# Joao-M-Silva/padel_analytics

Hardware: AMD Instinct MI355X
Metric: frames/sec (all trackers) on 1280x720 (higher is better)
Workload: dtype f32-equivalent (h2: fp16 pairs h + m/2048, 2 or 3 f16 MFMA products per multiply, fp32 accumulate)

## Files before the change

padel_analytics_amd/csrc/conv_1x1_h2s.hip:

```cpp
#include "h2_common.h"

namespace padel {

namespace {

__device__ __forceinline__ unsigned hs_off(int p, int q) { return (unsigned)(p * 64 + ((q ^ (((p >> 2) & 1) << 1)) << 4)); }

typedef int hs_i32x4 __attribute__((ext_vector_type(4)));

}

#ifndef PADEL_HS_AWIN
#define PADEL_HS_AWIN D
#endif
template <int WC, int PROBE = 0, int D = 2, int WR = 2>
__global__ void __launch_bounds__(64 * WR * WC, 2) conv_h2s_kernel(const ConvArgs a) {
    constexpr int MF = 4, NF = 3, NSET = D + 1;
    constexpr int kSPlaneB = 64 * WR * 64;
    constexpr int kSStageB = 2 * kSPlaneB;
    constexpr int kSStages = WC == 2 ? 5 : 9;
    constexpr int kSAhead = kSStages - 1;
    constexpr int NA = 8 / (2 * WC) * 2;
    static_assert(WR == 2 || WC == 4, "64-pixel tiles: one span per wave");
    __shared__ __attribute__((aligned(16))) float lds[(kSStages * kSStageB) / 4];
    char* const ldsb = reinterpret_cast<char*>(lds);
    const int tid = threadIdx.x;
    const int lane = tid & 63;
    const int wave = __builtin_amdgcn_readfirstlane(tid >> 6);
    const int wr = WR == 2 ? (wave & 1) : 0, wc = WR == 2 ? (wave >> 1) : wave;
    const int lr = lane & 15, lq = lane >> 4;

    const int nmt = a.n_mtiles, nnt = a.n_ntiles;
    const int bid = blockIdx.x;
    const int q8 = nmt >> 3, r8 = nmt & 7, xcd = bid & 7, idx = bid >> 3;
    const int mloc = idx / nnt, nt = idx - mloc * nnt;
    if (mloc >= q8 + (xcd < r8 ? 1 : 0)) return;
    const int mt = (xcd < r8 ? xcd * (q8 + 1) : r8 * (q8 + 1) + (xcd - r8) * q8) + mloc;
    const int m0 = mt * (64 * WR);
    const int f0 = nt * WC * NF;
    const int nch = a.cin >> 5;

    const long long pix_b = (long long)a.in_cs * 4;
    const char* const in0 = reinterpret_cast<const char*>(a.in + a.in_choff) + (long long)m0 * pix_b;
    i32x4 rsrcA = make_rsrc3(in0);
    {
        const long long left = ((long long)a.M - m0) * pix_b;
        rsrcA[2] = (int)(left > 0x7FFFFFFFll ? 0x7FFFFFFFll : left);
    }
    const int p_q = (lane & 3) ^ (((lane >> 4) & 1) << 1);
    const unsigned p_piece = (unsigned)((p_q >> 1) * 64 + (p_q & 1) * 16);
    unsigned voA[2];
#pragma unroll
    for (int k = 0; k < 2; ++k) voA[k] = (unsigned)(((wave + 4 * k) * 16 + (lane >> 2)) * (unsigned)pix_b) + p_piece;
    unsigned voL[2];
#pragma unroll
    for (int k = 0; k < 2; ++k) voL[k] = (unsigned)((wave * 16 + 8 * k + (lane >> 3)) * (unsigned)pix_b) + (unsigned)(lane & 7) * 16u;
    hs_i32x4 sink[2] = {};
    unsigned voQ[2];
#pragma unroll
    for (int k = 0; k < 2; ++k) voQ[k] = (unsigned)(wave * 2048 + k * 1024 + lane * 16);
    const unsigned lp0 = __builtin_amdgcn_readfirstlane((unsigned)(uintptr_t)lds);
    const unsigned lpw = __builtin_amdgcn_readfirstlane(lp0 + (unsigned)wave * 1024u);
#define PADEL_HS_REQA(SB_, K_)                                                                                    \
    if constexpr (PROBE != 3) {                                                                                   \
        const unsigned so_ = (unsigned)(K_) * 128u;                                                               \
        const unsigned lb_ = lpw + (unsigned)(SB_);                                                               \
        i32x4 rs_ = rsrcA;                                                                                        \
        if ((int)(K_) >= nch) rs_[2] = 0;                                                                         \
        if constexpr (PROBE == 4) { dma3<0>(voL[0], rs_, so_, lb_); dma3<kSPlaneB>(voL[1], rs_, so_, lb_); }      \
        else if constexpr (PROBE == 6) {                                                                          \
            asm volatile("buffer_load_dwordx4 %0, %1, %2, %3 offen" : "=v"(sink[0]) : "v"(voA[0]), "s"(rs_), "s"(so_) : "memory"); \
            asm volatile("buffer_load_dwordx4 %0, %1, %2, %3 offen" : "=v"(sink[1]) : "v"(voA[0]), "s"(rs_), "s"(so_ + 32u) : "memory"); \
        }                                                                                                         \
        else if constexpr (PROBE == 5) { dma3<0>(voQ[0], rs_, so_ * 128u, lb_); dma3<kSPlaneB>(voQ[1], rs_, so_ * 128u, lb_); } \
        else {                                                                                                    \
        dma3<0>(voA[0], rs_, so_, lb_); if constexpr (WC == 2) dma3<4096>(voA[1], rs_, so_, lb_);                 \
        dma3<kSPlaneB>(voA[0], rs_, so_ + 32u, lb_); if constexpr (WC == 2) dma3<kSPlaneB + 4096>(voA[1], rs_, so_ + 32u, lb_); \
        }                                                                                                         \
    }

    const unsigned fragb = (unsigned)nch * 2048u;
    const unsigned voffW = (unsigned)lane * 16u;
    i32x4 rsrcW[NF];
#pragma unroll
    for (int j = 0; j < NF; ++j) {
        const int frag = min(f0 + NF * wc + j, a.n16 - 1);
        rsrcW[j] = make_rsrc3(reinterpret_cast<const char*>(a.wr) + (long long)frag * fragb);
    }
    hs_i32x4 w[NSET][NF];
#define PADEL_HS_LOADW(SET_, K_)                                                                                  \
    if constexpr (PROBE != 2 && PROBE < 4 || PROBE == 7) {                                                        \
        const unsigned so_ = (unsigned)(K_) * 2048u;                                                              \
        if (PROBE == 7 && wr == 1) rsrcW[0][2] = rsrcW[1][2] = rsrcW[2][2] = 0;      \
        _Pragma("unroll") for (int j = 0; j < NF; ++j)                                                            \
            asm volatile("buffer_load_dwordx4 %0, %1, %2, %3 offen" : "=v"(w[SET_][j]) : "v"(voffW), "s"(rsrcW[j]), "s"(so_) : "memory"); \
    }
#define PADEL_HS_WAITW(SET_, N_)                                                                                  \
    asm volatile("s_waitcnt vmcnt(%3)" : "+v"(w[SET_][0]), "+v"(w[SET_][1]), "+v"(w[SET_][2]) : "n"(PROBE == 2 || (PROBE >= 4 && PROBE != 7) ? ((N_) == 0 ? 0 : (PADEL_HS_AWIN) * NA) : PROBE == 3 ? (N_) * NF / (NF + NA) : (N_)) : "memory")

    const unsigned abase = hs_off(64 * wr + lr, lq);
    f32x4 acc[MF][NF], part[MF][NF], cross[MF][NF];
#pragma unroll
    for (int f = 0; f < MF; ++f)
#pragma unroll
        for (int j = 0; j < NF; ++j) { acc[f][j] = (f32x4){0.f, 0.f, 0.f, 0.f}; part[f][j] = acc[f][j]; cross[f][j] = acc[f][j]; }
    h16x8 ah[MF], am[MF];
#define PADEL_HS_MFMA(F_, SET_)                                                                                   \
    do {                                                                                                          \
        _Pragma("unroll") for (int j = 0; j < NF; ++j)                                                            \
            cross[F_][j] = __builtin_amdgcn_mfma_f32_16x16x32_f16(__builtin_bit_cast(h16x8, w[SET_][j]), am[F_], cross[F_][j], 0, 0, 0); \
        _Pragma("unroll") for (int j = 0; j < NF; ++j)                                                            \
            part[F_][j] = __builtin_amdgcn_mfma_f32_16x16x32_f16(__builtin_bit_cast(h16x8, w[SET_][j]), ah[F_], part[F_][j], 0, 0, 0); \
        __builtin_amdgcn_sched_barrier(0);                                                                        \
    } while (0)
#define PADEL_HS_STEP(K_, SET_)                                                                                   \
    do {                                                                                                          \
        PADEL_HS_LOADW(((SET_) + D) % NSET, (K_) + D);                                                            \
        PADEL_HS_WAITW(SET_, D * (NF + NA));                                                                      \
        __builtin_amdgcn_s_barrier();              \
        asm volatile("" ::: "memory");                                                                            \
        PADEL_HS_REQA(s_wr, (K_) + kSAhead);                                                                      \
        __builtin_amdgcn_sched_barrier(0);                                                                        \
        if constexpr (PROBE == 0) {                                                                               \
            const char* p_ = ldsb + abase + s_rd;                                                                 \
            _Pragma("unroll") for (int f = 0; f < MF; ++f) {                                                      \
                ah[f] = *reinterpret_cast<const h16x8*>(p_ + f * 1024);                                           \
                am[f] = *reinterpret_cast<const h16x8*>(p_ + f * 1024 + kSPlaneB);                                \
            }                                                                                                     \
        }                                                                                                         \
        __builtin_amdgcn_sched_barrier(0);                                                                        \
        if constexpr (PROBE == 0) { PADEL_HS_MFMA(0, SET_); PADEL_HS_MFMA(1, SET_); PADEL_HS_MFMA(2, SET_); PADEL_HS_MFMA(3, SET_); } \
        if (++kblk == 9) {                         \
            kblk = 0;                                                                                             \
            _Pragma("unroll") for (int f = 0; f < MF; ++f)                                                        \
                _Pragma("unroll") for (int j = 0; j < NF; ++j) { acc[f][j] += part[f][j]; part[f][j] = (f32x4){0.f, 0.f, 0.f, 0.f}; } \
        }                                                                                                         \
        s_wr = s_rd;                                                                                              \
        s_rd = s_rd + (unsigned)kSStageB == (unsigned)(kSStages * kSStageB) ? 0u : s_rd + (unsigned)kSStageB;     \
    } while (0)

    int kblk = 0;
    unsigned s_rd = 0, s_wr = (unsigned)((kSStages - 1) * kSStageB);
    static_assert(kSAhead >= D, "the ring is at least as deep as the weight look-ahead");
#pragma unroll
    for (int k = 0; k < kSAhead - D; ++k) PADEL_HS_REQA(k * kSStageB, k);
#pragma unroll
    for (int i = 0; i < D; ++i) {
        PADEL_HS_LOADW(i, i);
        PADEL_HS_REQA((kSAhead - D + i) * kSStageB, kSAhead - D + i);
    }
#pragma unroll 1
    for (int k = 0; k < nch; k += NSET) {
        PADEL_HS_STEP(k, 0);
#pragma unroll
        for (int i = 1; i < NSET; ++i)
            if (k + i < nch) PADEL_HS_STEP(k + i, i);
    }
    if (kblk != 0) {
#pragma unroll
        for (int f = 0; f < MF; ++f)
#pragma unroll
            for (int j = 0; j < NF; ++j) acc[f][j] += part[f][j];
    }
#pragma unroll
    for (int i = 0; i < NSET; ++i) PADEL_HS_WAITW(i, 0);
    if constexpr (PROBE == 6) asm volatile("" :: "v"(sink[0]), "v"(sink[1]));
#undef PADEL_HS_STEP
#undef PADEL_HS_MFMA
#undef PADEL_HS_WAITW
#undef PADEL_HS_LOADW
#undef PADEL_HS_REQA

    int mpix[MF];
#pragma unroll
    for (int f = 0; f < MF; ++f) {
        const int m = m0 + 64 * wr + 16 * f + lr;
        mpix[f] = m < a.M ? m : -1;
    }
    const int fw = f0 + NF * wc;
    const bool fast = m0 + 64 * WR <= a.M && (fw + NF) * 16 <= a.cout && (((a.out_choff | a.out_cs) & 3) == 0) &&
                      (!a.res || (((a.res_choff | a.res_cs) & 3) == 0));
    if (fw < a.n16) h2_epilogue<MF, NF>(a, acc, cross, mpix, fw, lq, fast);
}

template <int PROBE = 0, int WR = 2>
__global__ void __launch_bounds__(256 * WR, 2) conv_h2s3_kernel(const ConvArgs a) {
    constexpr int MF = 4, NF = 3, WC = 4;
    constexpr int kSPlaneB = 64 * WR * 64, kSStageB = 2 * kSPlaneB;
    constexpr int kSStages = 9, kSAhead = 8, NA = 2;
    __shared__ __attribute__((aligned(16))) float lds[(kSStages * kSStageB) / 4];
    char* const ldsb = reinterpret_cast<char*>(lds);
    const int tid = threadIdx.x;
    const int lane = tid & 63;
    const int wave = __builtin_amdgcn_readfirstlane(tid >> 6);
    const int wr = WR == 2 ? (wave & 1) : 0, wc = WR == 2 ? (wave >> 1) : wave;
    const int lr = lane & 15, lq = lane >> 4;

    const int nmt = a.n_mtiles, nnt = a.n_ntiles;
    const int bid = blockIdx.x;
    const int q8 = nmt >> 3, r8 = nmt & 7, xcd = bid & 7, idx = bid >> 3;
    const int mloc = idx / nnt, nt = idx - mloc * nnt;
    if (mloc >= q8 + (xcd < r8 ? 1 : 0)) return;
    const int mt = (xcd < r8 ? xcd * (q8 + 1) : r8 * (q8 + 1) + (xcd - r8) * q8) + mloc;
    const int m0 = mt * (64 * WR);
    const int f0 = nt * WC * NF;
    const int nch = a.cin >> 5;
    const int HoWo = a.Ho * a.Wo;

    const long long pix_b = (long long)a.in_cs * 4;
    long long lin0;
    {
        const int n = fastdiv3(m0, a.howo_magic, a.howo_shift);
        const int rem = m0 - n * HoWo;
        const int oy = fastdiv3(rem, a.wo_magic, a.wo_shift), ox = rem - oy * a.Wo;
        lin0 = ((long long)n * a.H + (2 * oy - 1)) * a.W + (2 * ox - 1);
    }
    const i32x4 rsrcA = make_rsrc3(reinterpret_cast<const char*>(a.in + a.in_choff) + lin0 * pix_b);
    const int p_q = (lane & 3) ^ (((lane >> 4) & 1) << 1);
    const unsigned p_piece = (unsigned)((p_q >> 1) * 64 + (p_q & 1) * 16);
    unsigned voA, vbits = 0;
    {
        const int m = m0 + wave * 16 + (lane >> 2);
        const bool mv = m < a.M;
        const int mc = mv ? m : m0;
        const int n = fastdiv3(mc, a.howo_magic, a.howo_shift);
        const int rem = mc - n * HoWo;
        const int oy = fastdiv3(rem, a.wo_magic, a.wo_shift), ox = rem - oy * a.Wo;
        const int iy0 = 2 * oy - 1, ix0 = 2 * ox - 1;
        const long long lin = ((long long)n * a.H + iy0) * a.W + ix0;
        voA = (unsigned)((lin - lin0) * pix_b) + p_piece;
        if (mv) {
#pragma unroll
            for (int k = 0; k < 3; ++k) {
                vbits |= ((unsigned)(iy0 + k) < (unsigned)a.H ? 1u : 0u) << k;
                vbits |= ((unsigned)(ix0 + k) < (unsigned)a.W ? 8u : 0u) << k;
            }
        }
    }
    const unsigned rowb = (unsigned)a.W * (unsigned)pix_b;
    const unsigned lp0 = __builtin_amdgcn_readfirstlane((unsigned)(uintptr_t)lds);
    const unsigned lpw = __builtin_amdgcn_readfirstlane(lp0 + (unsigned)wave * 1024u);
#define PADEL_HS3_REQA(SB_, CH_, TAP_)                                                                            \
    do {                                                                                                          \
        constexpr int ky_ = (TAP_) % 3, kx_ = (TAP_) / 3;                                                         \
        constexpr unsigned need_ = (1u << ky_) | (8u << kx_);                                                     \
        const unsigned so_ = (unsigned)(CH_) * 128u + (unsigned)ky_ * rowb + (unsigned)kx_ * (unsigned)pix_b;     \
        const unsigned lb_ = lpw + (unsigned)(SB_);                                                               \
        i32x4 rs_ = rsrcA;                                                                                        \
        if ((int)(CH_) >= nch) rs_[2] = 0;                                                                        \
        const unsigned vo_ = (vbits & need_) == need_ ? voA : kOOR3;                                              \
        dma3<0>(vo_, rs_, so_, lb_); dma3<kSPlaneB>(vo_, rs_, so_ + 32u, lb_);                                    \
    } while (0)

    const unsigned fragb = (unsigned)(nch * 9) * 2048u;
    const unsigned voffW = (unsigned)lane * 16u;
    i32x4 rsrcW[NF];
#pragma unroll
    for (int j = 0; j < NF; ++j) {
        const int frag = min(f0 + NF * wc + j, a.n16 - 1);
        rsrcW[j] = make_rsrc3(reinterpret_cast<const char*>(a.wr) + (long long)frag * fragb);
    }
    hs_i32x4 w[3][NF];
    unsigned s_kw = 0;
#define PADEL_HS3_LOADW(SET_, TT_)                                                                                \
    do {                                                                                                          \
        const unsigned so_ = s_kw + (unsigned)((TT_) * 2048);                                                     \
        _Pragma("unroll") for (int j = 0; j < NF; ++j)                                                            \
            asm volatile("buffer_load_dwordx4 %0, %1, %2, %3 offen" : "=v"(w[SET_][j]) : "v"(voffW), "s"(rsrcW[j]), "s"(so_) : "memory"); \
    } while (0)
#define PADEL_HS3_WAITW(SET_, N_)                                                                                 \
    asm volatile("s_waitcnt vmcnt(%3)" : "+v"(w[SET_][0]), "+v"(w[SET_][1]), "+v"(w[SET_][2]) : "n"(N_) : "memory")

    const unsigned abase = hs_off(64 * wr + lr, lq);
    f32x4 acc[MF][NF], part[MF][NF], cross[MF][NF];
#pragma unroll
    for (int f = 0; f < MF; ++f)
#pragma unroll
        for (int j = 0; j < NF; ++j) { acc[f][j] = (f32x4){0.f, 0.f, 0.f, 0.f}; part[f][j] = acc[f][j]; cross[f][j] = acc[f][j]; }
    h16x8 ah[MF], am[MF];
#define PADEL_HS3_MFMA(F_, SET_)                                                                                  \
    do {                                                                                                          \
        _Pragma("unroll") for (int j = 0; j < NF; ++j)                                                            \
            cross[F_][j] = __builtin_amdgcn_mfma_f32_16x16x32_f16(__builtin_bit_cast(h16x8, w[SET_][j]), am[F_], cross[F_][j], 0, 0, 0); \
        _Pragma("unroll") for (int j = 0; j < NF; ++j)                                                            \
            part[F_][j] = __builtin_amdgcn_mfma_f32_16x16x32_f16(__builtin_bit_cast(h16x8, w[SET_][j]), ah[F_], part[F_][j], 0, 0, 0); \
        __builtin_amdgcn_sched_barrier(0);                                                                        \
    } while (0)
#define PADEL_HS3_STEP(T_)                                                                                        \
    do {                                                                                                          \
        PADEL_HS3_LOADW(((T_) + 2) % 3, (T_) + 2);                                                                \
        PADEL_HS3_WAITW((T_) % 3, 2 * NF + 2 * NA);                                                               \
        __builtin_amdgcn_s_barrier();                                                                             \
        asm volatile("" ::: "memory");                                                                            \
        PADEL_HS3_REQA(s_wr, c + ((T_) >= 1 ? 1 : 0), ((T_) + 8) % 9);                                            \
        __builtin_amdgcn_sched_barrier(0);                                                                        \
        if constexpr (PROBE == 0) {                                                                               \
            const char* p_ = ldsb + abase + s_rd;                                                                 \
            _Pragma("unroll") for (int f = 0; f < MF; ++f) {                                                      \
                ah[f] = *reinterpret_cast<const h16x8*>(p_ + f * 1024);                                           \
                am[f] = *reinterpret_cast<const h16x8*>(p_ + f * 1024 + kSPlaneB);                                \
            }                                                                                                     \
        }                                                                                                         \
        __builtin_amdgcn_sched_barrier(0);                                                                        \
        if constexpr (PROBE == 0) { PADEL_HS3_MFMA(0, (T_) % 3); PADEL_HS3_MFMA(1, (T_) % 3); PADEL_HS3_MFMA(2, (T_) % 3); PADEL_HS3_MFMA(3, (T_) % 3); } \
        s_wr = s_rd;                                                                                              \
        s_rd = s_rd + (unsigned)kSStageB == (unsigned)(kSStages * kSStageB) ? 0u : s_rd + (unsigned)kSStageB;     \
    } while (0)

    unsigned s_rd = 0, s_wr = (unsigned)((kSStages - 1) * kSStageB);
    PADEL_HS3_REQA(0 * kSStageB, 0, 0); PADEL_HS3_REQA(1 * kSStageB, 0, 1);
    PADEL_HS3_REQA(4 * kSStageB, 0, 4); PADEL_HS3_REQA(5 * kSStageB, 0, 5); PADEL_HS3_REQA(6 * kSStageB, 0, 6); PADEL_HS3_REQA(7 * kSStageB, 0, 7);
    PADEL_HS3_LOADW(0, 0);
    PADEL_HS3_REQA(2 * kSStageB, 0, 2);
    PADEL_HS3_LOADW(1, 1);
    PADEL_HS3_REQA(3 * kSStageB, 0, 3);
#pragma unroll 1
    for (int c = 0; c < nch; ++c) {
        PADEL_HS3_STEP(0); PADEL_HS3_STEP(1); PADEL_HS3_STEP(2); PADEL_HS3_STEP(3); PADEL_HS3_STEP(4);
        PADEL_HS3_STEP(5); PADEL_HS3_STEP(6); PADEL_HS3_STEP(7); PADEL_HS3_STEP(8);
#pragma unroll
        for (int f = 0; f < MF; ++f)
#pragma unroll
            for (int j = 0; j < NF; ++j) { acc[f][j] += part[f][j]; part[f][j] = (f32x4){0.f, 0.f, 0.f, 0.f}; }
        s_kw += 9u * 2048u;
    }
    PADEL_HS3_WAITW(0, 0); PADEL_HS3_WAITW(1, 0); PADEL_HS3_WAITW(2, 0);
#undef PADEL_HS3_STEP
#undef PADEL_HS3_MFMA
#undef PADEL_HS3_WAITW
#undef PADEL_HS3_LOADW
#undef PADEL_HS3_REQA

    int mpix[MF];
#pragma unroll
    for (int f = 0; f < MF; ++f) {
        const int m = m0 + 64 * wr + 16 * f + lr;
        mpix[f] = m < a.M ? m : -1;
    }
    const int fw = f0 + NF * wc;
    const bool fast = m0 + 64 * WR <= a.M && (fw + NF) * 16 <= a.cout && (((a.out_choff | a.out_cs) & 3) == 0) &&
                      (!a.res || (((a.res_choff | a.res_cs) & 3) == 0));
    if (fw < a.n16) h2_epilogue<MF, NF>(a, acc, cross, mpix, fw, lq, fast);
}

bool conv_h2s3_supported(const ConvArgs& a) {
    return a.w_single && a.wr && a.ksize == 3 && a.stride == 2 && (a.cin & 31) == 0 && a.cin >= 32 && a.w != nullptr && !a.in2 &&
           a.Ho <= (a.H + 1) / 2 && a.Wo <= (a.W + 1) / 2 && (long long)4 * a.W * a.in_cs * 4 < 0x3FFFFFFFll;
}

hipError_t launch_conv_h2s3(const ConvArgs& a_in, hipStream_t s, bool m64) {
    if (!conv_h2s3_supported(a_in)) return hipErrorNotSupported;
    ConvArgs a = a_in;
    a.n_mtiles = m64 ? (a.M + 63) / 64 : (a.M + 127) / 128;
    a.n_ntiles = (a.n16 + 11) / 12;
    dim3 grid(8u * (unsigned)((a.n_mtiles + 7) / 8) * (unsigned)a.n_ntiles, 1, 1);
    if (m64) {
        if (a.tune & 64) hipLaunchKernelGGL((conv_h2s3_kernel<1, 1>), grid, dim3(256), 0, s, a);
        else hipLaunchKernelGGL((conv_h2s3_kernel<0, 1>), grid, dim3(256), 0, s, a);
        return hipGetLastError();
    }
    if (a.tune & 64) hipLaunchKernelGGL((conv_h2s3_kernel<1>), grid, dim3(512), 0, s, a);
    else hipLaunchKernelGGL((conv_h2s3_kernel<0>), grid, dim3(512), 0, s, a);
    return hipGetLastError();
}

bool conv_h2s_supported(const ConvArgs& a) {
    return a.w_single && a.wr && a.ksize == 1 && a.stride == 1 && (a.cin & 31) == 0 && a.cin >= 64 && a.Ho == a.H && a.Wo == a.W && a.w != nullptr &&
           !a.in2 && (long long)128 * a.in_cs * 4 < 0x7FFFFFFFll;
}

hipError_t launch_conv_h2s(const ConvArgs& a_in, bool nf12, hipStream_t s, bool m64) {
    if (!conv_h2s_supported(a_in)) return hipErrorNotSupported;
    ConvArgs a = a_in;
    if (nf12 && m64) {
        a.n_mtiles = (a.M + 63) / 64;
        a.n_ntiles = (a.n16 + 11) / 12;
        dim3 grid(8u * (unsigned)((a.n_mtiles + 7) / 8) * (unsigned)a.n_ntiles, 1, 1);
        if (a.tune & 64) hipLaunchKernelGGL((conv_h2s_kernel<4, 1, 2, 1>), grid, dim3(256), 0, s, a);
        else hipLaunchKernelGGL((conv_h2s_kernel<4, 0, 2, 1>), grid, dim3(256), 0, s, a);
        return hipGetLastError();
    }
    a.n_mtiles = (a.M + 127) / 128;
    const bool wide = nf12;
    a.n_ntiles = wide ? (a.n16 + 11) / 12 : (a.n16 + 5) / 6;
    dim3 grid(8u * (unsigned)((a.n_mtiles + 7) / 8) * (unsigned)a.n_ntiles, 1, 1);
    if (wide) {
        static bool attr = false;
        if (!attr) {
            (void)hipFuncSetAttribute(reinterpret_cast<const void*>(conv_h2s_kernel<4, 0>), hipFuncAttributeMaxDynamicSharedMemorySize, 0);
            attr = true;
        }
        if ((a.tune & 64) && (a.tune & 4096)) hipLaunchKernelGGL((conv_h2s_kernel<4, 7>), grid, dim3(512), 0, s, a);
        else if ((a.tune & 64) && (a.tune & 2048)) hipLaunchKernelGGL((conv_h2s_kernel<4, 6>), grid, dim3(512), 0, s, a);
        else if ((a.tune & 64) && (a.tune & 1024)) hipLaunchKernelGGL((conv_h2s_kernel<4, 5>), grid, dim3(512), 0, s, a);
        else if ((a.tune & 64) && (a.tune & 256) && (a.tune & 512)) hipLaunchKernelGGL((conv_h2s_kernel<4, 4>), grid, dim3(512), 0, s, a);
        else if ((a.tune & 64) && (a.tune & 256)) hipLaunchKernelGGL((conv_h2s_kernel<4, 2>), grid, dim3(512), 0, s, a);
        else if ((a.tune & 64) && (a.tune & 512)) hipLaunchKernelGGL((conv_h2s_kernel<4, 3>), grid, dim3(512), 0, s, a);
        else if (a.tune & 64) hipLaunchKernelGGL((conv_h2s_kernel<4, 1>), grid, dim3(512), 0, s, a);
        else if (a.tune & 8) hipLaunchKernelGGL((conv_h2s_kernel<4, 0, 4>), grid, dim3(512), 0, s, a);
        else hipLaunchKernelGGL((conv_h2s_kernel<4, 0, 2>), grid, dim3(512), 0, s, a);
    } else if (a.tune & 64) hipLaunchKernelGGL((conv_h2s_kernel<2, 1>), grid, dim3(256), 0, s, a);
    else if (a.tune & 8) hipLaunchKernelGGL((conv_h2s_kernel<2, 0, 3>), grid, dim3(256), 0, s, a);
    else hipLaunchKernelGGL((conv_h2s_kernel<2, 0, 2>), grid, dim3(256), 0, s, a);
    return hipGetLastError();
}

}
```

padel_analytics_amd/csrc/conv_patch_h2v.hip:

```cpp
#include "h2_common.h"

namespace padel {

namespace {

constexpr int kVPW = 18, kVNPix = 18 * 18;
constexpr int kVSpans = (kVNPix + 15) / 16;
constexpr int kVPlaneB = kVSpans * 1024;
constexpr int kVTSpans = (kVNPix + 31) / 32;
constexpr int kVTPlaneB = kVTSpans * 1024;

__device__ __forceinline__ unsigned hv_tail_off(int p, int s) { return (unsigned)(p * 32 + ((s ^ ((p >> 3) & 1)) << 4)); }

typedef int hv_i32x4 __attribute__((ext_vector_type(4)));

}

template <int NF, bool CHUNK, bool TAIL, bool WS>
__global__ void __launch_bounds__(256, 2) conv_h2v_kernel(const ConvArgs a) {
    static_assert(CHUNK || TAIL, "cin = 32 CHUNK + 16 TAIL");
    static_assert(WS || NF <= 2, "three products: 2 fragments per wave (6 register sets of 4 VGPRs per step)");
    constexpr int MF = 4;
    constexpr int PATCH_B = (CHUNK ? 2 * kVPlaneB : 0);
    constexpr int TPATCH_B = (TAIL ? 2 * kVTPlaneB : 0);
    constexpr int NSTEPS = (CHUNK ? 9 : 0) + (TAIL ? 5 : 0);
    constexpr int NPL = WS ? 1 : 2;
    constexpr int NW = NF * NPL;
    __shared__ __attribute__((aligned(16))) float lds[(PATCH_B + TPATCH_B) / 4];
    char* const ldsb = reinterpret_cast<char*>(lds);
    const int tid = threadIdx.x;
    const int lane = tid & 63;
    const int wave = __builtin_amdgcn_readfirstlane(tid >> 6);
    const int lr = lane & 15, lq = lane >> 4;

    const int nmt = a.n_mtiles, nnt = a.n_ntiles;
    const int bid = blockIdx.x;
    const int q8 = nmt >> 3, r8 = nmt & 7, xcd = bid & 7, idx = bid >> 3;
    const int mloc = idx / nnt, nt = idx - mloc * nnt;
    if (mloc >= q8 + (xcd < r8 ? 1 : 0)) return;
    const int mt = (xcd < r8 ? xcd * (q8 + 1) : r8 * (q8 + 1) + (xcd - r8) * q8) + mloc;
    const int txN = (a.Wo + 15) >> 4, tyN = (a.Ho + 15) >> 4;
    const int tpi = tyN * txN;
    const int n = mt / tpi, rt = mt - n * tpi;
    const int ty = rt / txN, tx = rt - ty * txN;
    const int y0 = ty * 16, x0 = tx * 16;
    const int f0 = nt * NF;

    const float* const in0 = a.in + (((long long)n * a.H + (y0 - 1)) * a.W + (x0 - 1)) * a.in_cs + a.in_choff;
    const i32x4 rsrcP = make_rsrc3(in0);
    const unsigned lp0 = __builtin_amdgcn_readfirstlane((unsigned)(uintptr_t)lds);

    if constexpr (CHUNK) {
        const int p_lane = lane >> 2;
        const int p_q = (lane & 3) ^ (((lane >> 4) & 1) << 1);
        const unsigned p_piece = (unsigned)((p_q >> 1) * 64 + (p_q & 1) * 16);
#define PADEL_HV_PSPAN(S_)                                                                                        \
        if (((S_) & 3) == wave) {                                                                                 \
            const int pp_ = (S_) * 16 + p_lane;                                                                   \
            const int py_ = pp_ / kVPW, px_ = pp_ - py_ * kVPW;                                                   \
            const bool ok_ = pp_ < kVNPix && (unsigned)(y0 - 1 + py_) < (unsigned)a.H && (unsigned)(x0 - 1 + px_) < (unsigned)a.W; \
            const unsigned vo_ = ok_ ? (unsigned)((py_ * a.W + px_) * a.in_cs * 4) + p_piece : kOOR3;             \
            dma3<(S_) * 1024>(vo_, rsrcP, 0u, lp0);                                                               \
            dma3<kVPlaneB + (S_) * 1024>(vo_, rsrcP, 32u, lp0);                                                   \
        }
        PADEL_HV_PSPAN(0) PADEL_HV_PSPAN(1) PADEL_HV_PSPAN(2) PADEL_HV_PSPAN(3) PADEL_HV_PSPAN(4) PADEL_HV_PSPAN(5) PADEL_HV_PSPAN(6)
        PADEL_HV_PSPAN(7) PADEL_HV_PSPAN(8) PADEL_HV_PSPAN(9) PADEL_HV_PSPAN(10) PADEL_HV_PSPAN(11) PADEL_HV_PSPAN(12) PADEL_HV_PSPAN(13)
        PADEL_HV_PSPAN(14) PADEL_HV_PSPAN(15) PADEL_HV_PSPAN(16) PADEL_HV_PSPAN(17) PADEL_HV_PSPAN(18) PADEL_HV_PSPAN(19) PADEL_HV_PSPAN(20)
#undef PADEL_HV_PSPAN
    }
    if constexpr (TAIL) {
        const int t_lane = lane >> 1;
        const unsigned t_piece = (unsigned)(((lane & 1) ^ ((lane >> 4) & 1)) * 16);
        const unsigned t_so = CHUNK ? 128u : 0u;
#define PADEL_HV_TSPAN(S_)                                                                                        \
        if (((S_) & 3) == ((wave + 1) & 3)) {                                                                     \
            const int pp_ = (S_) * 32 + t_lane;                                                                   \
            const int py_ = pp_ / kVPW, px_ = pp_ - py_ * kVPW;                                                   \
            const bool ok_ = pp_ < kVNPix && (unsigned)(y0 - 1 + py_) < (unsigned)a.H && (unsigned)(x0 - 1 + px_) < (unsigned)a.W; \
            const unsigned vo_ = ok_ ? (unsigned)((py_ * a.W + px_) * a.in_cs * 4) + t_piece : kOOR3;             \
            dma3<PATCH_B + (S_) * 1024>(vo_, rsrcP, t_so, lp0);                                                   \
            dma3<PATCH_B + kVTPlaneB + (S_) * 1024>(vo_, rsrcP, t_so + 32u, lp0);                                 \
        }
        PADEL_HV_TSPAN(0) PADEL_HV_TSPAN(1) PADEL_HV_TSPAN(2) PADEL_HV_TSPAN(3) PADEL_HV_TSPAN(4) PADEL_HV_TSPAN(5)
        PADEL_HV_TSPAN(6) PADEL_HV_TSPAN(7) PADEL_HV_TSPAN(8) PADEL_HV_TSPAN(9) PADEL_HV_TSPAN(10)
#undef PADEL_HV_TSPAN
    }

    constexpr unsigned fragb = (unsigned)NSTEPS * 2048u;
    const unsigned voffW = (unsigned)lane * 16u;
    i32x4 rsrcW[NF];
#pragma unroll
    for (int j = 0; j < NF; ++j) {
        const int frag = min(f0 + j, a.n16 - 1);
        rsrcW[j] = make_rsrc3(reinterpret_cast<const char*>(a.wr) + (long long)frag * fragb);
    }
    hv_i32x4 w[3][NF], wm[3][WS ? 1 : NF];
#define PADEL_HV_LOADW(ST_)                                                                                       \
    do {                                                                                                          \
        const unsigned so_ = (unsigned)((ST_) * 2048);                                                            \
        _Pragma("unroll") for (int j = 0; j < NF; ++j) {                                                          \
            asm volatile("buffer_load_dwordx4 %0, %1, %2, %3 offen"                                               \
                         : "=v"(w[(ST_) % 3][j]) : "v"(voffW), "s"(rsrcW[j]), "s"(so_) : "memory");               \
            if constexpr (!WS)                                                                                    \
                asm volatile("buffer_load_dwordx4 %0, %1, %2, %3 offen offset:1024"                               \
                             : "=v"(wm[(ST_) % 3][j]) : "v"(voffW), "s"(rsrcW[j]), "s"(so_) : "memory");          \
        }                                                                                                         \
    } while (0)
#define PADEL_HV_WAITW(ST_, N_)                                                                                   \
    do {                                                                                                          \
        if constexpr (NF == 3)                                                                                    \
            asm volatile("s_waitcnt vmcnt(%3)" : "+v"(w[(ST_) % 3][0]), "+v"(w[(ST_) % 3][1]), "+v"(w[(ST_) % 3][2]) : "n"(N_) : "memory"); \
        else if constexpr (NF == 2 && WS)                                                                         \
            asm volatile("s_waitcnt vmcnt(%2)" : "+v"(w[(ST_) % 3][0]), "+v"(w[(ST_) % 3][1]) : "n"(N_) : "memory"); \
        else if constexpr (NF == 2)                                                                               \
            asm volatile("s_waitcnt vmcnt(%4)" : "+v"(w[(ST_) % 3][0]), "+v"(w[(ST_) % 3][1]), "+v"(wm[(ST_) % 3][0]), "+v"(wm[(ST_) % 3][WS ? 0 : NF - 1]) \
                         : "n"(N_) : "memory");                                                                   \
        else if constexpr (WS)                                                                                    \
            asm volatile("s_waitcnt vmcnt(%1)" : "+v"(w[(ST_) % 3][0]) : "n"(N_) : "memory");                     \
        else                                                                                                      \
            asm volatile("s_waitcnt vmcnt(%2)" : "+v"(w[(ST_) % 3][0]), "+v"(wm[(ST_) % 3][0]) : "n"(N_) : "memory"); \
    } while (0)

    unsigned rbase[8];
    if constexpr (CHUNK) {
#pragma unroll
        for (int r = 0; r < 8; ++r) {
            const int p0 = 4 * wave * kVPW + lr;
            rbase[r] = (unsigned)(p0 * 64 + ((lq ^ ((((p0 + r) >> 2) & 1) << 1)) << 4));
        }
    }
    const int rd_pix = 4 * wave * kVPW + lr;

    f32x4 acc[MF][NF], part[MF][NF], cross[MF][NF];
#pragma unroll
    for (int f = 0; f < MF; ++f)
#pragma unroll
        for (int j = 0; j < NF; ++j) { acc[f][j] = (f32x4){0.f, 0.f, 0.f, 0.f}; part[f][j] = acc[f][j]; cross[f][j] = acc[f][j]; }
    h16x8 ah[4], am[4];
#define PADEL_HV_READROW(R_, KX_)                                                                                 \
    do {                                                                                                          \
        constexpr int d_ = (R_) * kVPW + (KX_);                                                                   \
        const char* p_ = ldsb + rbase[d_ & 7];                                                                    \
        ah[(R_) & 3] = *reinterpret_cast<const h16x8*>(p_ + d_ * 64);                                             \
        am[(R_) & 3] = *reinterpret_cast<const h16x8*>(p_ + d_ * 64 + kVPlaneB);                                  \
    } while (0)
#define PADEL_HV_MFMA_ROW(F_, S_, ST_)                                                                            \
    do {                                                                                                          \
        _Pragma("unroll") for (int j = 0; j < NF; ++j)                                                            \
            cross[F_][j] = __builtin_amdgcn_mfma_f32_16x16x32_f16(__builtin_bit_cast(h16x8, w[(ST_) % 3][j]), am[S_], cross[F_][j], 0, 0, 0); \
        if constexpr (!WS) {                                                                                      \
            _Pragma("unroll") for (int j = 0; j < NF; ++j)                                                        \
                cross[F_][j] = __builtin_amdgcn_mfma_f32_16x16x32_f16(__builtin_bit_cast(h16x8, wm[(ST_) % 3][WS ? 0 : j]), ah[S_], cross[F_][j], 0, 0, 0); \
        }                                                                                                         \
        _Pragma("unroll") for (int j = 0; j < NF; ++j)                                                            \
            part[F_][j] = __builtin_amdgcn_mfma_f32_16x16x32_f16(__builtin_bit_cast(h16x8, w[(ST_) % 3][j]), ah[S_], part[F_][j], 0, 0, 0); \
        __builtin_amdgcn_sched_barrier(0);                                                                        \
    } while (0)
#define PADEL_HV_TOP(ST_)                                                                                         \
    do {                                                                                                          \
        if constexpr ((ST_) + 2 < NSTEPS) PADEL_HV_LOADW((ST_) + 2);                                              \
        PADEL_HV_WAITW(ST_, NW * (((ST_) + 1 < NSTEPS ? 1 : 0) + ((ST_) + 2 < NSTEPS ? 1 : 0)));                  \
        __builtin_amdgcn_sched_barrier(0);                                                                        \
    } while (0)
#define PADEL_HV_STEP(T_)                                                                                         \
    do {                                                                                                          \
        constexpr int kx_ = h2_tap_kx(T_), ky_ = h2_tap_ky(T_);                                                   \
        PADEL_HV_TOP(T_);                                                                                         \
        if constexpr (ky_ == 0) {                                                                                 \
            PADEL_HV_MFMA_ROW(0, 0, T_);                                                                          \
            PADEL_HV_READROW(4, kx_);                                                                             \
            __builtin_amdgcn_sched_barrier(0);                                                                    \
            PADEL_HV_MFMA_ROW(1, 1, T_); PADEL_HV_MFMA_ROW(2, 2, T_); PADEL_HV_MFMA_ROW(3, 3, T_);                \
        } else if constexpr (ky_ == 1) {                                                                          \
            PADEL_HV_MFMA_ROW(0, 1, T_);                                                                          \
            PADEL_HV_READROW(5, kx_);                                                                             \
            __builtin_amdgcn_sched_barrier(0);                                                                    \
            PADEL_HV_MFMA_ROW(1, 2, T_); PADEL_HV_MFMA_ROW(2, 3, T_); PADEL_HV_MFMA_ROW(3, 0, T_);                \
        } else {                                            \
            PADEL_HV_MFMA_ROW(2, 0, T_);                                                                          \
            if constexpr (kx_ < 2) PADEL_HV_READROW(0, kx_ + 1);                                                  \
            __builtin_amdgcn_sched_barrier(0);                                                                    \
            PADEL_HV_MFMA_ROW(3, 1, T_);                                                                          \
            if constexpr (kx_ < 2) PADEL_HV_READROW(1, kx_ + 1);                                                  \
            __builtin_amdgcn_sched_barrier(0);                                                                    \
            PADEL_HV_MFMA_ROW(0, 2, T_);                                                                          \
            if constexpr (kx_ < 2) PADEL_HV_READROW(2, kx_ + 1);                                                  \
            __builtin_amdgcn_sched_barrier(0);                                                                    \
            PADEL_HV_MFMA_ROW(1, 3, T_);                                                                          \
            if constexpr (kx_ < 2) PADEL_HV_READROW(3, kx_ + 1);                                                  \
            __builtin_amdgcn_sched_barrier(0);                                                                    \
        }                                                                                                         \
    } while (0)
#define PADEL_HV_TSTEP(JT_, ST_)                                                                                  \
    do {                                                                                                          \
        constexpr int ta_ = 2 * (JT_), tb_ = 2 * (JT_) + 1 < 9 ? 2 * (JT_) + 1 : 8;                               \
        int rp_ = rd_pix;                                                                                         \
        asm volatile("" : "+v"(rp_));                                                                             \
        _Pragma("unroll") for (int f = 0; f < MF; ++f) {                                                          \
            const int pa_ = rp_ + (f + h2_tap_ky(ta_)) * kVPW + h2_tap_kx(ta_), pb_ = rp_ + (f + h2_tap_ky(tb_)) * kVPW + h2_tap_kx(tb_); \
            const char* p_ = ldsb + PATCH_B + hv_tail_off((lq >> 1) ? pb_ : pa_, lq & 1);                         \
            ah[f] = *reinterpret_cast<const h16x8*>(p_);                                                          \
            am[f] = *reinterpret_cast<const h16x8*>(p_ + kVTPlaneB);                                              \
        }                                                                                                         \
        __builtin_amdgcn_sched_barrier(0);                                                                        \
        PADEL_HV_TOP(ST_);                                                                                        \
        PADEL_HV_MFMA_ROW(0, 0, ST_); PADEL_HV_MFMA_ROW(1, 1, ST_); PADEL_HV_MFMA_ROW(2, 2, ST_); PADEL_HV_MFMA_ROW(3, 3, ST_); \
    } while (0)
#define PADEL_HV_FLUSH()                                                                                          \
    do {                                                                                                          \
        _Pragma("unroll") for (int f = 0; f < MF; ++f)                                                            \
            _Pragma("unroll") for (int j = 0; j < NF; ++j) { acc[f][j] += part[f][j]; part[f][j] = (f32x4){0.f, 0.f, 0.f, 0.f}; } \
    } while (0)

    PADEL_HV_LOADW(0);
    if constexpr (NSTEPS > 1) PADEL_HV_LOADW(1);
    wait_vm3<NW * (NSTEPS > 1 ? 2 : 1)>();
    __builtin_amdgcn_s_barrier();
    asm volatile("" ::: "memory");
    if constexpr (CHUNK) {
        PADEL_HV_READROW(0, 0); PADEL_HV_READROW(1, 0); PADEL_HV_READROW(2, 0); PADEL_HV_READROW(3, 0);
        __builtin_amdgcn_sched_barrier(0);
        PADEL_HV_STEP(0); PADEL_HV_STEP(1); PADEL_HV_STEP(2); PADEL_HV_STEP(3); PADEL_HV_STEP(4);
        PADEL_HV_STEP(5); PADEL_HV_STEP(6); PADEL_HV_STEP(7); PADEL_HV_STEP(8);
        PADEL_HV_FLUSH();
    }
    if constexpr (TAIL) {
        constexpr int S0 = CHUNK ? 9 : 0;
        PADEL_HV_TSTEP(0, S0); PADEL_HV_TSTEP(1, S0 + 1); PADEL_HV_TSTEP(2, S0 + 2); PADEL_HV_TSTEP(3, S0 + 3); PADEL_HV_TSTEP(4, S0 + 4);
        PADEL_HV_FLUSH();
    }
#undef PADEL_HV_FLUSH
#undef PADEL_HV_TSTEP
#undef PADEL_HV_STEP
#undef PADEL_HV_TOP
#undef PADEL_HV_MFMA_ROW
#undef PADEL_HV_READROW
#undef PADEL_HV_WAITW
#undef PADEL_HV_LOADW

    int mpix[MF];
#pragma unroll
    for (int f = 0; f < MF; ++f) {
        const int oy = y0 + 4 * wave + f, ox = x0 + lr;
        mpix[f] = (oy < a.Ho && ox < a.Wo) ? (n * a.Ho + oy) * a.Wo + ox : -1;
    }
    const bool fast = y0 + 16 <= a.Ho && x0 + 16 <= a.Wo && (f0 + NF) * 16 <= a.cout && (((a.out_choff | a.out_cs) & 3) == 0) &&
                      (!a.res || (((a.res_choff | a.res_cs) & 3) == 0));
    h2_epilogue<MF, NF>(a, acc, cross, mpix, f0, lq, fast);
}

bool conv_h2v_supported(const ConvArgs& a) {
    return a.wr && a.ksize == 3 && a.stride == 1 && (a.cin == 16 || a.cin == 32 || a.cin == 48) && a.Ho == a.H && a.Wo == a.W && a.w != nullptr && !a.in2;
}

template <int NF, bool WS>
static hipError_t launch_hv(const ConvArgs& a_in, hipStream_t s) {
    ConvArgs a = a_in;
    const int batch = a.M / (a.Ho * a.Wo);
    a.n_mtiles = batch * ((a.Ho + 15) / 16) * ((a.Wo + 15) / 16);
    a.n_ntiles = (a.n16 + NF - 1) / NF;
    dim3 grid(8u * (unsigned)((a.n_mtiles + 7) / 8) * (unsigned)a.n_ntiles, 1, 1);
    if (a.cin == 48) hipLaunchKernelGGL((conv_h2v_kernel<NF, true, true, WS>), grid, dim3(256), 0, s, a);
    else if (a.cin == 32) hipLaunchKernelGGL((conv_h2v_kernel<NF, true, false, WS>), grid, dim3(256), 0, s, a);
    else hipLaunchKernelGGL((conv_h2v_kernel<NF, false, true, WS>), grid, dim3(256), 0, s, a);
    return hipGetLastError();
}

hipError_t launch_conv_h2v(const ConvArgs& a, int nf, hipStream_t s) {
    if (!conv_h2v_supported(a)) return hipErrorNotSupported;
    if (a.w_single) {
        switch (nf) {
            case 1: return launch_hv<1, true>(a, s);
            case 2: return launch_hv<2, true>(a, s);
            case 3: return launch_hv<3, true>(a, s);
        }
    } else {
        switch (nf) {
            case 1: return launch_hv<1, false>(a, s);
            case 2: return launch_hv<2, false>(a, s);
        }
    }
    return hipErrorNotSupported;
}

}
```

padel_analytics_amd/csrc/h2_common.h:

```cpp
#pragma once
#include "bx3_common.h"
#include "act_fast.h"

namespace padel {

typedef _Float16 h16x8 __attribute__((ext_vector_type(8)));
typedef _Float16 h16x4 __attribute__((ext_vector_type(4)));

namespace {

constexpr float kH2Max = 65504.0f;
constexpr float kH2Scale = 2048.0f, kH2InvScale = 1.0f / 2048.0f;
constexpr unsigned kOORh = 0x80000000u;

__host__ __device__ constexpr int h2_tap_ky(int t) { return t % 3; }
__host__ __device__ constexpr int h2_tap_kx(int t) { return t / 3; }

__device__ __forceinline__ long long h2_chan_off(int c) { return (long long)(c >> 4) * 64 + (c & 15) * 2; }

typedef float h2_f32x2 __attribute__((ext_vector_type(2)));
typedef _Float16 h2_h16x2 __attribute__((ext_vector_type(2)));

__device__ __forceinline__ void h2_encode4(const f32x4 v, h16x4& h, h16x4& m, bool& bad) {
#pragma unroll
    for (int p = 0; p < 2; ++p) {
        bad = bad || !(fabsf(v[2 * p]) <= kH2Max) || !(fabsf(v[2 * p + 1]) <= kH2Max);
        const h2_f32x2 x = {__builtin_amdgcn_fmed3f(v[2 * p], -kH2Max, kH2Max), __builtin_amdgcn_fmed3f(v[2 * p + 1], -kH2Max, kH2Max)};
        const h2_h16x2 hh = __builtin_convertvector(x, h2_h16x2);
        const h2_f32x2 rr = {(x[0] - (float)hh[0]) * kH2Scale, (x[1] - (float)hh[1]) * kH2Scale};
        const h2_h16x2 mm = __builtin_convertvector(rr, h2_h16x2);
        h[2 * p] = hh[0]; h[2 * p + 1] = hh[1];
        m[2 * p] = mm[0]; m[2 * p + 1] = mm[1];
    }
}

template <int ACT>
__device__ __forceinline__ float h2_act(float x) { return fast_act<ACT>(x); }
__device__ __forceinline__ f32x4 h2_decode4(const h16x4 h, const h16x4 m) {
    f32x4 v;
#pragma unroll
    for (int r = 0; r < 4; ++r) v[r] = fmaf((float)m[r], kH2InvScale, (float)h[r]);
    return v;
}
__device__ __forceinline__ void h2_raise(unsigned* flag, bool bad) {
    if (__builtin_amdgcn_ballot_w64(bad) != 0ull && (threadIdx.x & 63) == 0) atomicOr(flag, 1u);
}

}

typedef unsigned h2_u32x4 __attribute__((ext_vector_type(4)));
typedef unsigned h2_u32x2 __attribute__((ext_vector_type(2)));
typedef unsigned short h2_u16x2 __attribute__((ext_vector_type(2)));

__device__ __forceinline__ float h2_conv_value(float cross, float mainacc, float sc, float b) {
    return fmaf(fmaf(cross, kH2InvScale, mainacc), sc, b);
}
__device__ __forceinline__ f32x4 h2_residual4(const h2_u32x4 rr) {
    const h2_u32x2 s0 = __builtin_amdgcn_permlane16_swap(rr[0], rr[2], false, false);
    const h2_u32x2 s1 = __builtin_amdgcn_permlane16_swap(rr[1], rr[3], false, false);
    const h2_u32x2 hd = {s0[0], s1[0]}, md = {s0[1], s1[1]};
    return h2_decode4(__builtin_bit_cast(h16x4, hd), __builtin_bit_cast(h16x4, md));
}

template <int MF, int NF, int ACT, bool RES, bool F32OUT>
__device__ __forceinline__ void h2_epilogue_fast(const ConvArgs& a, const f32x4 (&mainacc)[MF][NF], const f32x4 (&cross)[MF][NF],
                                                 const int (&mpix)[MF], int fw, int lq, bool& bad) {
    static_assert(!(RES && F32OUT), "fp32 head maps have no residual");
    f32x4 b[NF], sc[NF];
#pragma unroll
    for (int j = 0; j < NF; ++j) {
        const int co0 = (fw + j) * 16 + lq * 4;
        b[j] = *reinterpret_cast<const f32x4*>(a.bias + co0);
        sc[j] = *reinterpret_cast<const f32x4*>(a.oscale + co0);
    }
    if constexpr (F32OUT) {
        float* op[MF];
#pragma unroll
        for (int f = 0; f < MF; ++f) op[f] = a.out + (long long)mpix[f] * a.out_cs + (a.out_choff + fw * 16 + lq * 4);
#pragma unroll
        for (int j = 0; j < NF; ++j)
#pragma unroll
            for (int f = 0; f < MF; ++f) {
                f32x4 v;
#pragma unroll
                for (int r = 0; r < 4; ++r) v[r] = h2_act<ACT>(h2_conv_value(cross[f][j][r], mainacc[f][j][r], sc[j][r], b[j][r]));
                *reinterpret_cast<f32x4*>(op[f] + j * 16) = v;
            }
    } else {
        const int piece = ((lq & 1) << 5) | ((lq >> 1) << 4);
        char* op[MF];
        h2_u32x4 rr[MF][NF];
#pragma unroll
        for (int f = 0; f < MF; ++f) {
            op[f] = reinterpret_cast<char*>(a.out) + (long long)mpix[f] * a.out_cs * 4 + ((((a.out_choff >> 4) + fw) << 6) + piece);
            if constexpr (RES) {
                const char* rp = reinterpret_cast<const char*>(a.res) + (long long)mpix[f] * a.res_cs * 4 + ((((a.res_choff >> 4) + fw) << 6) + piece);
#pragma unroll
                for (int j = 0; j < NF; ++j) rr[f][j] = *reinterpret_cast<const h2_u32x4*>(rp + j * 64);
            }
        }
        h2_u16x2 top = {0, 0};
#pragma unroll
        for (int j = 0; j < NF; ++j)
#pragma unroll
            for (int f = 0; f < MF; ++f) {
                f32x4 v;
#pragma unroll
                for (int r = 0; r < 4; ++r) v[r] = h2_conv_value(cross[f][j][r], mainacc[f][j][r], sc[j][r], b[j][r]);
                if constexpr (RES) {
                    const f32x4 rv = h2_residual4(rr[f][j]);
                    if (a.res_pre) {
#pragma unroll
                        for (int r = 0; r < 4; ++r) v[r] = h2_act<ACT>(v[r] + rv[r]);
                    } else {
#pragma unroll
                        for (int r = 0; r < 4; ++r) v[r] = h2_act<ACT>(v[r]) + rv[r];
                    }
                } else {
#pragma unroll
                    for (int r = 0; r < 4; ++r) v[r] = h2_act<ACT>(v[r]);
                }
                h2_u32x2 hd, md;
#pragma unroll
                for (int p = 0; p < 2; ++p) {
                    const h2_f32x2 x = {__builtin_amdgcn_fmed3f(v[2 * p], -kH2Max, kH2Max), __builtin_amdgcn_fmed3f(v[2 * p + 1], -kH2Max, kH2Max)};
                    const h2_h16x2 hh = __builtin_convertvector(x, h2_h16x2);
                    const h2_f32x2 res = {(x[0] - (float)hh[0]) * kH2Scale, (x[1] - (float)hh[1]) * kH2Scale};
                    const h2_h16x2 mm = __builtin_convertvector(res, h2_h16x2);
                    hd[p] = __builtin_bit_cast(unsigned, hh);
                    md[p] = __builtin_bit_cast(unsigned, mm);
                    top = __builtin_elementwise_max(top, __builtin_bit_cast(h2_u16x2, hd[p] & 0x7FFF7FFFu));
                }
                const h2_u32x2 s0 = __builtin_amdgcn_permlane16_swap(hd[0], md[0], false, false);
                const h2_u32x2 s1 = __builtin_amdgcn_permlane16_swap(hd[1], md[1], false, false);
                const h2_u32x4 o = {s0[0], s1[0], s0[1], s1[1]};
                *reinterpret_cast<h2_u32x4*>(op[f] + j * 64) = o;
            }
        bad = bad || top[0] >= 0x7BFFu || top[1] >= 0x7BFFu;
    }
}

template <int MF, int NF, int ACT, bool RES>
__device__ __forceinline__ void h2_epilogue_slow(const ConvArgs& a, const f32x4 (&mainacc)[MF][NF], const f32x4 (&cross)[MF][NF],
                                                 const int (&mpix)[MF], int fw, int lq, bool& bad) {
    char* const outb = reinterpret_cast<char*>(a.out);
    const char* const resb = reinterpret_cast<const char*>(a.res);
#pragma unroll
    for (int j = 0; j < NF; ++j) {
        const int co0 = (fw + j) * 16 + lq * 4;
        f32x4 b, sc;
#pragma unroll
        for (int r = 0; r < 4; ++r) { b[r] = a.bias[min(co0 + r, a.n16 * 16 - 1)]; sc[r] = a.oscale[min(co0 + r, a.n16 * 16 - 1)]; }
#pragma unroll
        for (int f = 0; f < MF; ++f) {
            const int m = mpix[f];
            if (m < 0) continue;
#pragma unroll
            for (int r = 0; r < 4; ++r) {
                const int co = co0 + r;
                if (co >= a.cout) continue;
                float x = h2_conv_value(cross[f][j][r], mainacc[f][j][r], sc[r], b[r]);
                if (RES) {
                    const int rc = a.res_choff + co;
                    const _Float16* rp = reinterpret_cast<const _Float16*>(resb + (long long)m * a.res_cs * 4 + (long long)(rc >> 4) * 64) + (rc & 15);
                    const float rv = fmaf((float)rp[16], kH2InvScale, (float)rp[0]);
                    x = a.res_pre ? h2_act<ACT>(x + rv) : h2_act<ACT>(x) + rv;
                } else {
                    x = h2_act<ACT>(x);
                }
                if (a.out_f32) {
                    a.out[(long long)m * a.out_cs + a.out_choff + co] = x;
                } else {
                    bad |= !(fabsf(x) <= kH2Max);
                    const float xc = __builtin_amdgcn_fmed3f(x, -kH2Max, kH2Max);
                    const _Float16 hh = (_Float16)xc;
                    const int oc = a.out_choff + co;
                    _Float16* op = reinterpret_cast<_Float16*>(outb + (long long)m * a.out_cs * 4 + (long long)(oc >> 4) * 64) + (oc & 15);
                    op[0] = hh;
                    op[16] = (_Float16)((xc - (float)hh) * kH2Scale);
                }
            }
        }
    }
}

template <int MF, int NF>
__device__ __forceinline__ void h2_epilogue(const ConvArgs& a, const f32x4 (&mainacc)[MF][NF], const f32x4 (&cross)[MF][NF],
                                            const int (&mpix)[MF], int fw, int lq, bool fast) {
    const bool wide = fast && (a.out_f32 ? !a.res : ((((a.out_choff | a.out_cs) & 15) == 0) && (!a.res || (((a.res_choff | a.res_cs) & 15) == 0))));
    bool bad = false;
#define PADEL_H2_EPI(ACT_)                                                                                        \
    do {                                                                                                          \
        if (wide) {                                                                                               \
            if (a.out_f32) h2_epilogue_fast<MF, NF, ACT_, false, true>(a, mainacc, cross, mpix, fw, lq, bad);     \
            else if (a.res) h2_epilogue_fast<MF, NF, ACT_, true, false>(a, mainacc, cross, mpix, fw, lq, bad);    \
            else h2_epilogue_fast<MF, NF, ACT_, false, false>(a, mainacc, cross, mpix, fw, lq, bad);              \
        } else if (a.res) h2_epilogue_slow<MF, NF, ACT_, true>(a, mainacc, cross, mpix, fw, lq, bad);             \
        else h2_epilogue_slow<MF, NF, ACT_, false>(a, mainacc, cross, mpix, fw, lq, bad);                         \
    } while (0)
    if (a.act == ACT_SILU) PADEL_H2_EPI(ACT_SILU);
    else if (a.act == ACT_RELU) PADEL_H2_EPI(ACT_RELU);
    else if (a.act == ACT_SIGMOID) PADEL_H2_EPI(ACT_SIGMOID);
    else if (a.act == ACT_LEAKY) PADEL_H2_EPI(ACT_LEAKY);
    else PADEL_H2_EPI(ACT_NONE);
#undef PADEL_H2_EPI
    if (!a.out_f32) h2_raise(a.ovf_flag, bad);
}

}
```

Measured before the change: 1019.

## Make h2 conv kernels persistent and prefetch next tile's activations during epilogue

Turns the 1x1, stride-3 and h2v conv kernels into persistent kernels that walk several tiles with a grid-stride loop, with the grid sized from CU count times two slots. While the epilogue of the current tile runs, bias, scale and residual operands are loaded and pinned first, and then the first activation DMA stages for the next tile are issued. The aim is to hide the pipeline fill latency and the epilogue behind each other and to cut block launch and tail overhead. The cost is an extra barrier per tile and more register pressure, and walking is gated by tune bits and channel count in some paths.

```diff
diff --git a/padel_analytics_amd/csrc/conv_1x1_h2s.hip b/padel_analytics_amd/csrc/conv_1x1_h2s.hip
--- a/padel_analytics_amd/csrc/conv_1x1_h2s.hip
+++ b/padel_analytics_amd/csrc/conv_1x1_h2s.hip
@@ -7,14 +7,27 @@
 __device__ __forceinline__ unsigned hs_off(int p, int q) { return (unsigned)(p * 64 + ((q ^ (((p >> 2) & 1) << 1)) << 4)); }
 
 typedef int hs_i32x4 __attribute__((ext_vector_type(4)));
+
+struct HsTile { int m0, f0; bool valid; };
+__device__ __forceinline__ HsTile hs_tile(const ConvArgs& a, int v, int vmax, int bm, int frags_per_tile) {
+    HsTile t;
+    const int nmt = a.n_mtiles, nnt = a.n_ntiles;
+    const int q8 = nmt >> 3, r8 = nmt & 7, xcd = v & 7, idx = v >> 3;
+    const int mloc = idx / nnt, nt = idx - mloc * nnt;
+    t.valid = v < vmax && mloc < q8 + (xcd < r8 ? 1 : 0);
+    const int mt = (xcd < r8 ? xcd * (q8 + 1) : r8 * (q8 + 1) + (xcd - r8) * q8) + mloc;
+    t.m0 = mt * bm;
+    t.f0 = nt * frags_per_tile;
+    return t;
+}
 
 }
 
 #ifndef PADEL_HS_AWIN
 #define PADEL_HS_AWIN D
 #endif
-template <int WC, int PROBE = 0, int D = 2, int WR = 2>
-__global__ void __launch_bounds__(64 * WR * WC, 2) conv_h2s_kernel(const ConvArgs a) {
+template <int WC, int PROBE = 0, int D = 2, int WR = 2, bool WALK = false>
+__global__ void __launch_bounds__(64 * WR * WC, 2) conv_h2s_kernel(const ConvArgs a, const int vmax) {
     constexpr int MF = 4, NF = 3, NSET = D + 1;
     constexpr int kSPlaneB = 64 * WR * 64;
     constexpr int kSStageB = 2 * kSPlaneB;
@@ -30,23 +43,20 @@
     const int wr = WR == 2 ? (wave & 1) : 0, wc = WR == 2 ? (wave >> 1) : wave;
     const int lr = lane & 15, lq = lane >> 4;
 
-    const int nmt = a.n_mtiles, nnt = a.n_ntiles;
-    const int bid = blockIdx.x;
-    const int q8 = nmt >> 3, r8 = nmt & 7, xcd = bid & 7, idx = bid >> 3;
-    const int mloc = idx / nnt, nt = idx - mloc * nnt;
-    if (mloc >= q8 + (xcd < r8 ? 1 : 0)) return;
-    const int mt = (xcd < r8 ? xcd * (q8 + 1) : r8 * (q8 + 1) + (xcd - r8) * q8) + mloc;
-    const int m0 = mt * (64 * WR);
-    const int f0 = nt * WC * NF;
     const int nch = a.cin >> 5;
+    const int G = (int)gridDim.x;
+    int v = (int)blockIdx.x;
+    HsTile cur = hs_tile(a, v, vmax, 64 * WR, WC * NF);
+    if (!cur.valid) return;
 
     const long long pix_b = (long long)a.in_cs * 4;
-    const char* const in0 = reinterpret_cast<const char*>(a.in + a.in_choff) + (long long)m0 * pix_b;
-    i32x4 rsrcA = make_rsrc3(in0);
-    {
-        const long long left = ((long long)a.M - m0) * pix_b;
-        rsrcA[2] = (int)(left > 0x7FFFFFFFll ? 0x7FFFFFFFll : left);
-    }
+    i32x4 rsrcA, rsrcAn;
+#define PADEL_HS_RSRCA(RS_, T_)                                                                                   \
+    do {                                                                                                          \
+        RS_ = make_rsrc3(reinterpret_cast<const char*>(a.in + a.in_choff) + (long long)(T_).m0 * pix_b);          \
+        const long long left_ = ((long long)a.M - (T_).m0) * pix_b;                                               \
+        RS_[2] = (int)(left_ > 0x7FFFFFFFll ? 0x7FFFFFFFll : left_);                                              \
+    } while (0)
     const int p_q = (lane & 3) ^ (((lane >> 4) & 1) << 1);
     const unsigned p_piece = (unsigned)((p_q >> 1) * 64 + (p_q & 1) * 16);
     unsigned voA[2];
@@ -61,11 +71,11 @@
     for (int k = 0; k < 2; ++k) voQ[k] = (unsigned)(wave * 2048 + k * 1024 + lane * 16);
     const unsigned lp0 = __builtin_amdgcn_readfirstlane((unsigned)(uintptr_t)lds);
     const unsigned lpw = __builtin_amdgcn_readfirstlane(lp0 + (unsigned)wave * 1024u);
-#define PADEL_HS_REQA(SB_, K_)                                                                                    \
+#define PADEL_HS_REQA(SB_, K_, RS_)                                                                                  \
     if constexpr (PROBE != 3) {                                                                                   \
         const unsigned so_ = (unsigned)(K_) * 128u;                                                               \
         const unsigned lb_ = lpw + (unsigned)(SB_);                                                               \
-        i32x4 rs_ = rsrcA;                                                                                        \
+        i32x4 rs_ = RS_;                                                                                          \
         if ((int)(K_) >= nch) rs_[2] = 0;                                                                         \
         if constexpr (PROBE == 4) { dma3<0>(voL[0], rs_, so_, lb_); dma3<kSPlaneB>(voL[1], rs_, so_, lb_); }      \
         else if constexpr (PROBE == 6) {                                                                          \
@@ -82,11 +92,6 @@
     const unsigned fragb = (unsigned)nch * 2048u;
     const unsigned voffW = (unsigned)lane * 16u;
     i32x4 rsrcW[NF];
-#pragma unroll
-    for (int j = 0; j < NF; ++j) {
-        const int frag = min(f0 + NF * wc + j, a.n16 - 1);
-        rsrcW[j] = make_rsrc3(reinterpret_cast<const char*>(a.wr) + (long long)frag * fragb);
-    }
     hs_i32x4 w[NSET][NF];
 #define PADEL_HS_LOADW(SET_, K_)                                                                                  \
     if constexpr (PROBE != 2 && PROBE < 4 || PROBE == 7) {                                                        \
@@ -100,10 +105,6 @@
 
     const unsigned abase = hs_off(64 * wr + lr, lq);
     f32x4 acc[MF][NF], part[MF][NF], cross[MF][NF];
-#pragma unroll
-    for (int f = 0; f < MF; ++f)
-#pragma unroll
-        for (int j = 0; j < NF; ++j) { acc[f][j] = (f32x4){0.f, 0.f, 0.f, 0.f}; part[f][j] = acc[f][j]; cross[f][j] = acc[f][j]; }
     h16x8 ah[MF], am[MF];
 #define PADEL_HS_MFMA(F_, SET_)                                                                                   \
     do {                                                                                                          \
@@ -119,7 +120,7 @@
         PADEL_HS_WAITW(SET_, D * (NF + NA));                                                                      \
         __builtin_amdgcn_s_barrier();              \
         asm volatile("" ::: "memory");                                                                            \
-        PADEL_HS_REQA(s_wr, (K_) + kSAhead);                                                                      \
+        PADEL_HS_REQA(s_wr, (K_) + kSAhead, rsrcA);                                                                   \
         __builtin_amdgcn_sched_barrier(0);                                                                        \
         if constexpr (PROBE == 0) {                                                                               \
             const char* p_ = ldsb + abase + s_rd;                                                                 \
@@ -139,52 +140,92 @@
         s_rd = s_rd + (unsigned)kSStageB == (unsigned)(kSStages * kSStageB) ? 0u : s_rd + (unsigned)kSStageB;     \
     } while (0)
 
-    int kblk = 0;
-    unsigned s_rd = 0, s_wr = (unsigned)((kSStages - 1) * kSStageB);
     static_assert(kSAhead >= D, "the ring is at least as deep as the weight look-ahead");
-#pragma unroll
-    for (int k = 0; k < kSAhead - D; ++k) PADEL_HS_REQA(k * kSStageB, k);
-#pragma unroll
-    for (int i = 0; i < D; ++i) {
-        PADEL_HS_LOADW(i, i);
-        PADEL_HS_REQA((kSAhead - D + i) * kSStageB, kSAhead - D + i);
+#define PADEL_HS_FIRSTA(RS_)                                                                                      \
+    do {                                                                                                          \
+        _Pragma("unroll") for (int k = 0; k < kSAhead - D; ++k) PADEL_HS_REQA(k * kSStageB, k, RS_);              \
+    } while (0)
+    PADEL_HS_RSRCA(rsrcA, cur);
+    PADEL_HS_FIRSTA(rsrcA);
+    for (;;) {
+#pragma unroll
+        for (int j = 0; j < NF; ++j) {
+            const int frag = min(cur.f0 + NF * wc + j, a.n16 - 1);
+            rsrcW[j] = make_rsrc3(reinterpret_cast<const char*>(a.wr) + (long long)frag * fragb);
+        }
+#pragma unroll
+        for (int i = 0; i < D; ++i) {
+            PADEL_HS_LOADW(i, i);
+            PADEL_HS_REQA((kSAhead - D + i) * kSStageB, kSAhead - D + i, rsrcA);
+        }
+        HsTile nxt = {0, 0, false};
+        if constexpr (WALK) {
+            nxt = hs_tile(a, v + G, vmax, 64 * WR, WC * NF);
+            PADEL_HS_RSRCA(rsrcAn, nxt);
+        }
+#pragma unroll
+        for (int f = 0; f < MF; ++f)
+#pragma unroll
+            for (int j = 0; j < NF; ++j) { acc[f][j] = (f32x4){0.f, 0.f, 0.f, 0.f}; part[f][j] = acc[f][j]; cross[f][j] = acc[f][j]; }
+        int kblk = 0;
+        unsigned s_rd = 0, s_wr = (unsigned)((kSStages - 1) * kSStageB);
+#pragma unroll 1
+        for (int k = 0; k < nch; k += NSET) {
+            PADEL_HS_STEP(k, 0);
+#pragma unroll
+            for (int i = 1; i < NSET; ++i)
+                if (k + i < nch) PADEL_HS_STEP(k + i, i);
+        }
+        if (kblk != 0) {
+#pragma unroll
+            for (int f = 0; f < MF; ++f)
+#pragma unroll
+                for (int j = 0; j < NF; ++j) acc[f][j] += part[f][j];
+        }
+        int mpix[MF];
+#pragma unroll
+        for (int f = 0; f < MF; ++f) {
+            const int m = cur.m0 + 64 * wr + 16 * f + lr;
+            mpix[f] = m < a.M ? m : -1;
+        }
+        const int fw = cur.f0 + NF * wc;
+        const bool fast = cur.m0 + 64 * WR <= a.M && (fw + NF) * 16 <= a.cout && (((a.out_choff | a.out_cs) & 3) == 0) &&
+                          (!a.res || (((a.res_choff | a.res_cs) & 3) == 0));
+#pragma unroll
+        for (int i = 0; i < NSET; ++i) PADEL_HS_WAITW(i, 0);
+        if constexpr (PROBE == 6) asm volatile("" :: "v"(sink[0]), "v"(sink[1]));
+        if constexpr (WALK) {
+            if (nxt.valid) {
+                asm volatile("s_waitcnt lgkmcnt(0)" ::: "memory");
+                __builtin_amdgcn_s_barrier();
+                asm volatile("" ::: "memory");
+            }
+        }
+        if constexpr (WALK) {
+            const auto issue_next = [&]() {
+                if (nxt.valid) PADEL_HS_FIRSTA(rsrcAn);
+            };
+            if (fw < a.n16) h2_epilogue_walk<MF, NF>(a, acc, cross, mpix, fw, lq, fast, issue_next);
+            else issue_next();
+        } else {
+            if (fw < a.n16) h2_epilogue<MF, NF>(a, acc, cross, mpix, fw, lq, fast);
+        }
+        if (!WALK || !nxt.valid) break;
+        cur = nxt;
+        rsrcA = rsrcAn;
+        v += G;
     }
-#pragma unroll 1
-    for (int k = 0; k < nch; k += NSET) {
-        PADEL_HS_STEP(k, 0);
-#pragma unroll
-        for (int i = 1; i < NSET; ++i)
-            if (k + i < nch) PADEL_HS_STEP(k + i, i);
-    }
-    if (kblk != 0) {
-#pragma unroll
-        for (int f = 0; f < MF; ++f)
-#pragma unroll
-            for (int j = 0; j < NF; ++j) acc[f][j] += part[f][j];
-    }
-#pragma unroll
-    for (int i = 0; i < NSET; ++i) PADEL_HS_WAITW(i, 0);
-    if constexpr (PROBE == 6) asm volatile("" :: "v"(sink[0]), "v"(sink[1]));
+#undef PADEL_HS_FIRSTA
+#undef PADEL_HS_RSRCA
 #undef PADEL_HS_STEP
 #undef PADEL_HS_MFMA
 #undef PADEL_HS_WAITW
 #undef PADEL_HS_LOADW
 #undef PADEL_HS_REQA
-
-    int mpix[MF];
-#pragma unroll
-    for (int f = 0; f < MF; ++f) {
-        const int m = m0 + 64 * wr + 16 * f + lr;
-        mpix[f] = m < a.M ? m : -1;
-    }
-    const int fw = f0 + NF * wc;
-    const bool fast = m0 + 64 * WR <= a.M && (fw + NF) * 16 <= a.cout && (((a.out_choff | a.out_cs) & 3) == 0) &&
-                      (!a.res || (((a.res_choff | a.res_cs) & 3) == 0));
-    if (fw < a.n16) h2_epilogue<MF, NF>(a, acc, cross, mpix, fw, lq, fast);
-}
-
-template <int PROBE = 0, int WR = 2>
-__global__ void __launch_bounds__(256 * WR, 2) conv_h2s3_kernel(const ConvArgs a) {
+}
+
+template <int PROBE = 0, int WR = 2, bool WALK = false>
+__global__ void __launch_bounds__(256 * WR, 2) conv_h2s3_kernel(const ConvArgs a, const int vmax) {
     constexpr int MF = 4, NF = 3, WC = 4;
     constexpr int kSPlaneB = 64 * WR * 64, kSStageB = 2 * kSPlaneB;
     constexpr int kSStages = 9, kSAhead = 8, NA = 2;
@@ -196,70 +237,64 @@
     const int wr = WR == 2 ? (wave & 1) : 0, wc = WR == 2 ? (wave >> 1) : wave;
     const int lr = lane & 15, lq = lane >> 4;
 
-    const int nmt = a.n_mtiles, nnt = a.n_ntiles;
-    const int bid = blockIdx.x;
-    const int q8 = nmt >> 3, r8 = nmt & 7, xcd = bid & 7, idx = bid >> 3;
-    const int mloc = idx / nnt, nt = idx - mloc * nnt;
-    if (mloc >= q8 + (xcd < r8 ? 1 : 0)) return;
-    const int mt = (xcd < r8 ? xcd * (q8 + 1) : r8 * (q8 + 1) + (xcd - r8) * q8) + mloc;
-    const int m0 = mt * (64 * WR);
-    const int f0 = nt * WC * NF;
     const int nch = a.cin >> 5;
     const int HoWo = a.Ho * a.Wo;
+    const int G = (int)gridDim.x;
+    int v = (int)blockIdx.x;
+    HsTile cur = hs_tile(a, v, vmax, 64 * WR, WC * NF);
+    if (!cur.valid) return;
 
     const long long pix_b = (long long)a.in_cs * 4;
-    long long lin0;
-    {
-        const int n = fastdiv3(m0, a.howo_magic, a.howo_shift);
-        const int rem = m0 - n * HoWo;
-        const int oy = fastdiv3(rem, a.wo_magic, a.wo_shift), ox = rem - oy * a.Wo;
-        lin0 = ((long long)n * a.H + (2 * oy - 1)) * a.W + (2 * ox - 1);
-    }
-    const i32x4 rsrcA = make_rsrc3(reinterpret_cast<const char*>(a.in + a.in_choff) + lin0 * pix_b);
     const int p_q = (lane & 3) ^ (((lane >> 4) & 1) << 1);
     const unsigned p_piece = (unsigned)((p_q >> 1) * 64 + (p_q & 1) * 16);
-    unsigned voA, vbits = 0;
-    {
-        const int m = m0 + wave * 16 + (lane >> 2);
-        const bool mv = m < a.M;
-        const int mc = mv ? m : m0;
-        const int n = fastdiv3(mc, a.howo_magic, a.howo_shift);
-        const int rem = mc - n * HoWo;
-        const int oy = fastdiv3(rem, a.wo_magic, a.wo_shift), ox = rem - oy * a.Wo;
-        const int iy0 = 2 * oy - 1, ix0 = 2 * ox - 1;
-        const long long lin = ((long long)n * a.H + iy0) * a.W + ix0;
-        voA = (unsigned)((lin - lin0) * pix_b) + p_piece;
-        if (mv) {
-#pragma unroll
-            for (int k = 0; k < 3; ++k) {
-                vbits |= ((unsigned)(iy0 + k) < (unsigned)a.H ? 1u : 0u) << k;
-                vbits |= ((unsigned)(ix0 + k) < (unsigned)a.W ? 8u : 0u) << k;
-            }
-        }
-    }
+    i32x4 rsrcA, rsrcAn;
+    unsigned voA, vbits, voAn, vbitsn;
+#define PADEL_HS3_PARAMS(T_, RS_, VO_, VB_)                                                                       \
+    do {                                                                                                          \
+        const int m0_ = (T_).m0;                                                                                  \
+        long long lin0_;                                                                                          \
+        {                                                                                                         \
+            const int n = fastdiv3(m0_, a.howo_magic, a.howo_shift);                                              \
+            const int rem = m0_ - n * HoWo;                                                                       \
+            const int oy = fastdiv3(rem, a.wo_magic, a.wo_shift), ox = rem - oy * a.Wo;                           \
+            lin0_ = ((long long)n * a.H + (2 * oy - 1)) * a.W + (2 * ox - 1);                                     \
+        }                                                                                                         \
+        RS_ = make_rsrc3(reinterpret_cast<const char*>(a.in + a.in_choff) + lin0_ * pix_b);                       \
+        const int m = m0_ + wave * 16 + (lane >> 2);                                                              \
+        const bool mv = m < a.M;                                                                                  \
+        const int mc = mv ? m : m0_;                                                                              \
+        const int n = fastdiv3(mc, a.howo_magic, a.howo_shift);                                                   \
+        const int rem = mc - n * HoWo;                                                                            \
+        const int oy = fastdiv3(rem, a.wo_magic, a.wo_shift), ox = rem - oy * a.Wo;                               \
+        const int iy0 = 2 * oy - 1, ix0 = 2 * ox - 1;                                                             \
+        const long long lin = ((long long)n * a.H + iy0) * a.W + ix0;                                             \
+        VO_ = (unsigned)((lin - lin0_) * pix_b) + p_piece;                                                        \
+        VB_ = 0;                                                                                                  \
+        if (mv) {                                                                                                 \
+            _Pragma("unroll") for (int k = 0; k < 3; ++k) {                                                       \
+                VB_ |= ((unsigned)(iy0 + k) < (unsigned)a.H ? 1u : 0u) << k;                                      \
+                VB_ |= ((unsigned)(ix0 + k) < (unsigned)a.W ? 8u : 0u) << k;                                      \
+            }                                                                                                     \
+        }                                                                                                         \
+    } while (0)
     const unsigned rowb = (unsigned)a.W * (unsigned)pix_b;
     const unsigned lp0 = __builtin_amdgcn_readfirstlane((unsigned)(uintptr_t)lds);
     const unsigned lpw = __builtin_amdgcn_readfirstlane(lp0 + (unsigned)wave * 1024u);
-#define PADEL_HS3_REQA(SB_, CH_, TAP_)                                                                            \
+#define PADEL_HS3_REQA(SB_, CH_, TAP_, RS_, VO_, VB_)                                                                          \
     do {                                                                                                          \
         constexpr int ky_ = (TAP_) % 3, kx_ = (TAP_) / 3;                                                         \
         constexpr unsigned need_ = (1u << ky_) | (8u << kx_);                                                     \
         const unsigned so_ = (unsigned)(CH_) * 128u + (unsigned)ky_ * rowb + (unsigned)kx_ * (unsigned)pix_b;     \
         const unsigned lb_ = lpw + (unsigned)(SB_);                                                               \
-        i32x4 rs_ = rsrcA;                                                                                        \
+        i32x4 rs_ = RS_;                                                                                          \
         if ((int)(CH_) >= nch) rs_[2] = 0;                                                                        \
-        const unsigned vo_ = (vbits & need_) == need_ ? voA : kOOR3;                                              \
+        const unsigned vo_ = ((VB_) & need_) == need_ ? (VO_) : kOOR3;                                            \
         dma3<0>(vo_, rs_, so_, lb_); dma3<kSPlaneB>(vo_, rs_, so_ + 32u, lb_);                                    \
     } while (0)
 
     const unsigned fragb = (unsigned)(nch * 9) * 2048u;
     const unsigned voffW = (unsigned)lane * 16u;
     i32x4 rsrcW[NF];
-#pragma unroll
-    for (int j = 0; j < NF; ++j) {
-        const int frag = min(f0 + NF * wc + j, a.n16 - 1);
-        rsrcW[j] = make_rsrc3(reinterpret_cast<const char*>(a.wr) + (long long)frag * fragb);
-    }
     hs_i32x4 w[3][NF];
     unsigned s_kw = 0;
 #define PADEL_HS3_LOADW(SET_, TT_)                                                                                \
@@ -273,10 +308,6 @@
 
     const unsigned abase = hs_off(64 * wr + lr, lq);
     f32x4 acc[MF][NF], part[MF][NF], cross[MF][NF];
-#pragma unroll
-    for (int f = 0; f < MF; ++f)
-#pragma unroll
-        for (int j = 0; j < NF; ++j) { acc[f][j] = (f32x4){0.f, 0.f, 0.f, 0.f}; part[f][j] = acc[f][j]; cross[f][j] = acc[f][j]; }
     h16x8 ah[MF], am[MF];
 #define PADEL_HS3_MFMA(F_, SET_)                                                                                  \
     do {                                                                                                          \
@@ -292,7 +323,7 @@
         PADEL_HS3_WAITW((T_) % 3, 2 * NF + 2 * NA);                                                               \
         __builtin_amdgcn_s_barrier();                                                                             \
         asm volatile("" ::: "memory");                                                                            \
-        PADEL_HS3_REQA(s_wr, c + ((T_) >= 1 ? 1 : 0), ((T_) + 8) % 9);                                            \
+        PADEL_HS3_REQA(s_wr, c + ((T_) >= 1 ? 1 : 0), ((T_) + 8) % 9, rsrcA, voA, vbits);                        \
         __builtin_amdgcn_sched_barrier(0);                                                                        \
         if constexpr (PROBE == 0) {                                                                               \
             const char* p_ = ldsb + abase + s_rd;                                                                 \
@@ -307,40 +338,89 @@
         s_rd = s_rd + (unsigned)kSStageB == (unsigned)(kSStages * kSStageB) ? 0u : s_rd + (unsigned)kSStageB;     \
     } while (0)
 
-    unsigned s_rd = 0, s_wr = (unsigned)((kSStages - 1) * kSStageB);
-    PADEL_HS3_REQA(0 * kSStageB, 0, 0); PADEL_HS3_REQA(1 * kSStageB, 0, 1);
-    PADEL_HS3_REQA(4 * kSStageB, 0, 4); PADEL_HS3_REQA(5 * kSStageB, 0, 5); PADEL_HS3_REQA(6 * kSStageB, 0, 6); PADEL_HS3_REQA(7 * kSStageB, 0, 7);
-    PADEL_HS3_LOADW(0, 0);
-    PADEL_HS3_REQA(2 * kSStageB, 0, 2);
-    PADEL_HS3_LOADW(1, 1);
-    PADEL_HS3_REQA(3 * kSStageB, 0, 3);
+#define PADEL_HS3_FIRSTA(RS_, VO_, VB_)                                                                           \
+    do {                                                                                                          \
+        PADEL_HS3_REQA(0 * kSStageB, 0, 0, RS_, VO_, VB_); PADEL_HS3_REQA(1 * kSStageB, 0, 1, RS_, VO_, VB_);     \
+        PADEL_HS3_REQA(4 * kSStageB, 0, 4, RS_, VO_, VB_); PADEL_HS3_REQA(5 * kSStageB, 0, 5, RS_, VO_, VB_);     \
+        PADEL_HS3_REQA(6 * kSStageB, 0, 6, RS_, VO_, VB_); PADEL_HS3_REQA(7 * kSStageB, 0, 7, RS_, VO_, VB_);     \
+    } while (0)
+    PADEL_HS3_PARAMS(cur, rsrcA, voA, vbits);
+    PADEL_HS3_FIRSTA(rsrcA, voA, vbits);
+    for (;;) {
+#pragma unroll
+        for (int j = 0; j < NF; ++j) {
+            const int frag = min(cur.f0 + NF * wc + j, a.n16 - 1);
+            rsrcW[j] = make_rsrc3(reinterpret_cast<const char*>(a.wr) + (long long)frag * fragb);
+        }
+        s_kw = 0;
+        PADEL_HS3_LOADW(0, 0);
+        PADEL_HS3_REQA(2 * kSStageB, 0, 2, rsrcA, voA, vbits);
+        PADEL_HS3_LOADW(1, 1);
+        PADEL_HS3_REQA(3 * kSStageB, 0, 3, rsrcA, voA, vbits);
+        HsTile nxt = {0, 0, false};
+        if constexpr (WALK) {
+            nxt = hs_tile(a, v + G, vmax, 64 * WR, WC * NF);
+            PADEL_HS3_PARAMS(nxt, rsrcAn, voAn, vbitsn);
+        }
+#pragma unroll
+        for (int f = 0; f < MF; ++f)
+#pragma unroll
+            for (int j = 0; j < NF; ++j) { acc[f][j] = (f32x4){0.f, 0.f, 0.f, 0.f}; part[f][j] = acc[f][j]; cross[f][j] = acc[f][j]; }
+        unsigned s_rd = 0, s_wr = (unsigned)((kSStages - 1) * kSStageB);
 #pragma unroll 1
-    for (int c = 0; c < nch; ++c) {
-        PADEL_HS3_STEP(0); PADEL_HS3_STEP(1); PADEL_HS3_STEP(2); PADEL_HS3_STEP(3); PADEL_HS3_STEP(4);
-        PADEL_HS3_STEP(5); PADEL_HS3_STEP(6); PADEL_HS3_STEP(7); PADEL_HS3_STEP(8);
-#pragma unroll
-        for (int f = 0; f < MF; ++f)
-#pragma unroll
-            for (int j = 0; j < NF; ++j) { acc[f][j] += part[f][j]; part[f][j] = (f32x4){0.f, 0.f, 0.f, 0.f}; }
-        s_kw += 9u * 2048u;
+        for (int c = 0; c < nch; ++c) {
+            PADEL_HS3_STEP(0); PADEL_HS3_STEP(1); PADEL_HS3_STEP(2); PADEL_HS3_STEP(3); PADEL_HS3_STEP(4);
+            PADEL_HS3_STEP(5); PADEL_HS3_STEP(6); PADEL_HS3_STEP(7); PADEL_HS3_STEP(8);
+#pragma unroll
+            for (int f = 0; f < MF; ++f)
+#pragma unroll
+                for (int j = 0; j < NF; ++j) { acc[f][j] += part[f][j]; part[f][j] = (f32x4){0.f, 0.f, 0.f, 0.f}; }
+            s_kw += 9u * 2048u;
+        }
+        int mpix[MF];
+#pragma unroll
+        for (int f = 0; f < MF; ++f) {
+            const int m = cur.m0 + 64 * wr + 16 * f + lr;
+            mpix[f] = m < a.M ? m : -1;
+        }
+        const int fw = cur.f0 + NF * wc;
+        const bool fast = cur.m0 + 64 * WR <= a.M && (fw + NF) * 16 <= a.cout && (((a.out_choff | a.out_cs) & 3) == 0) &&
+                          (!a.res || (((a.res_choff | a.res_cs) & 3) == 0));
+        PADEL_HS3_WAITW(0, 0); PADEL_HS3_WAITW(1, 0); PADEL_HS3_WAITW(2, 0);
+        if constexpr (WALK) {
+            if (nxt.valid) {
+                asm volatile("s_waitcnt lgkmcnt(0)" ::: "memory");
+                __builtin_amdgcn_s_barrier();
+                asm volatile("" ::: "memory");
+            }
+        }
+        if constexpr (WALK) {
+            const auto issue_next = [&]() {
+                if (nxt.valid) PADEL_HS3_FIRSTA(rsrcAn, voAn, vbitsn);
+            };
+            if (fw < a.n16) h2_epilogue_walk<MF, NF>(a, acc, cross, mpix, fw, lq, fast, issue_next);
+            else issue_next();
+        } else {
+            if (fw < a.n16) h2_epilogue<MF, NF>(a, acc, cross, mpix, fw, lq, fast);
+        }
+        if (!WALK || !nxt.valid) break;
+        cur = nxt;
+        rsrcA = rsrcAn; voA = voAn; vbits = vbitsn;
+        v += G;
     }
-    PADEL_HS3_WAITW(0, 0); PADEL_HS3_WAITW(1, 0); PADEL_HS3_WAITW(2, 0);
+#undef PADEL_HS3_FIRSTA
+#undef PADEL_HS3_PARAMS
 #undef PADEL_HS3_STEP
 #undef PADEL_HS3_MFMA
 #undef PADEL_HS3_WAITW
 #undef PADEL_HS3_LOADW
 #undef PADEL_HS3_REQA
-
-    int mpix[MF];
-#pragma unroll
-    for (int f = 0; f < MF; ++f) {
-        const int m = m0 + 64 * wr + 16 * f + lr;
-        mpix[f] = m < a.M ? m : -1;
-    }
-    const int fw = f0 + NF * wc;
-    const bool fast = m0 + 64 * WR <= a.M && (fw + NF) * 16 <= a.cout && (((a.out_choff | a.out_cs) & 3) == 0) &&
-                      (!a.res || (((a.res_choff | a.res_cs) & 3) == 0));
-    if (fw < a.n16) h2_epilogue<MF, NF>(a, acc, cross, mpix, fw, lq, fast);
+}
+
+static bool hs_walks(const ConvArgs& a, bool dflt) { return !(a.tune & 4) && (dflt || (a.tune & 16)); }
+static dim3 hs_walk_grid(int vmax, int per_cu, bool walk) {
+    const int per = walk ? h2_walk_slots(per_cu) : vmax;
+    return dim3((unsigned)(vmax < per ? vmax : per), 1, 1);
 }
 
 bool conv_h2s3_supported(const ConvArgs& a) {
@@ -353,14 +433,18 @@
     ConvArgs a = a_in;
     a.n_mtiles = m64 ? (a.M + 63) / 64 : (a.M + 127) / 128;
     a.n_ntiles = (a.n16 + 11) / 12;
-    dim3 grid(8u * (unsigned)((a.n_mtiles + 7) / 8) * (unsigned)a.n_ntiles, 1, 1);
+    const int vmax = 8 * ((a.n_mtiles + 7) / 8) * a.n_ntiles;
+    const bool walk = hs_walks(a, false) && !(a.tune & 64);
+    const dim3 grid = hs_walk_grid(vmax, m64 ? 2 : 1, walk);
     if (m64) {
-        if (a.tune & 64) hipLaunchKernelGGL((conv_h2s3_kernel<1, 1>), grid, dim3(256), 0, s, a);
-        else hipLaunchKernelGGL((conv_h2s3_kernel<0, 1>), grid, dim3(256), 0, s, a);
+        if (a.tune & 64) hipLaunchKernelGGL((conv_h2s3_kernel<1, 1>), grid, dim3(256), 0, s, a, vmax);
+        else if (walk) hipLaunchKernelGGL((conv_h2s3_kernel<0, 1, true>), grid, dim3(256), 0, s, a, vmax);
+        else hipLaunchKernelGGL((conv_h2s3_kernel<0, 1>), grid, dim3(256), 0, s, a, vmax);
         return hipGetLastError();
     }
-    if (a.tune & 64) hipLaunchKernelGGL((conv_h2s3_kernel<1>), grid, dim3(512), 0, s, a);
-    else hipLaunchKernelGGL((conv_h2s3_kernel<0>), grid, dim3(512), 0, s, a);
+    if (a.tune & 64) hipLaunchKernelGGL((conv_h2s3_kernel<1>), grid, dim3(512), 0, s, a, vmax);
+    else if (walk) hipLaunchKernelGGL((conv_h2s3_kernel<0, 2, true>), grid, dim3(512), 0, s, a, vmax);
+    else hipLaunchKernelGGL((conv_h2s3_kernel<0>), grid, dim3(512), 0, s, a, vmax);
     return hipGetLastError();
 }
 
@@ -375,33 +459,44 @@
     if (nf12 && m64) {
         a.n_mtiles = (a.M + 63) / 64;
         a.n_ntiles = (a.n16 + 11) / 12;
-        dim3 grid(8u * (unsigned)((a.n_mtiles + 7) / 8) * (unsigned)a.n_ntiles, 1, 1);
-        if (a.tune & 64) hipLaunchKernelGGL((conv_h2s_kernel<4, 1, 2, 1>), grid, dim3(256), 0, s, a);
-        else hipLaunchKernelGGL((conv_h2s_kernel<4, 0, 2, 1>), grid, dim3(256), 0, s, a);
+        const int vmax = 8 * ((a.n_mtiles + 7) / 8) * a.n_ntiles;
+        const bool walk = hs_walks(a, false) && !(a.tune & 64);
+        const dim3 grid = hs_walk_grid(vmax, 2, walk);
+        if (a.tune & 64) hipLaunchKernelGGL((conv_h2s_kernel<4, 1, 2, 1>), grid, dim3(256), 0, s, a, vmax);
+        else if (walk) hipLaunchKernelGGL((conv_h2s_kernel<4, 0, 2, 1, true>), grid, dim3(256), 0, s, a, vmax);
+        else hipLaunchKernelGGL((conv_h2s_kernel<4, 0, 2, 1>), grid, dim3(256), 0, s, a, vmax);
         return hipGetLastError();
     }
     a.n_mtiles = (a.M + 127) / 128;
     const bool wide = nf12;
     a.n_ntiles = wide ? (a.n16 + 11) / 12 : (a.n16 + 5) / 6;
-    dim3 grid(8u * (unsigned)((a.n_mtiles + 7) / 8) * (unsigned)a.n_ntiles, 1, 1);
+    const int vmax = 8 * ((a.n_mtiles + 7) / 8) * a.n_ntiles;
+    const bool walk = hs_walks(a, wide) && !(a.tune & 64);
+    const dim3 grid = hs_walk_grid(vmax, wide ? 1 : 2, walk);
     if (wide) {
         static bool attr = false;
         if (!attr) {
             (void)hipFuncSetAttribute(reinterpret_cast<const void*>(conv_h2s_kernel<4, 0>), hipFuncAttributeMaxDynamicSharedMemorySize, 0);
             attr = true;
         }
-        if ((a.tune & 64) && (a.tune & 4096)) hipLaunchKernelGGL((conv_h2s_kernel<4, 7>), grid, dim3(512), 0, s, a);
-        else if ((a.tune & 64) && (a.tune & 2048)) hipLaunchKernelGGL((conv_h2s_kernel<4, 6>), grid, dim3(512), 0, s, a);
-        else if ((a.tune & 64) && (a.tune & 1024)) hipLaunchKernelGGL((conv_h2s_kernel<4, 5>), grid, dim3(512), 0, s, a);
-        else if ((a.tune & 64) && (a.tune & 256) && (a.tune & 512)) hipLaunchKernelGGL((conv_h2s_kernel<4, 4>), grid, dim3(512), 0, s, a);
-        else if ((a.tune & 64) && (a.tune & 256)) hipLaunchKernelGGL((conv_h2s_kernel<4, 2>), grid, dim3(512), 0, s, a);
-        else if ((a.tune & 64) && (a.tune & 512)) hipLaunchKernelGGL((conv_h2s_kernel<4, 3>), grid, dim3(512), 0, s, a);
-        else if (a.tune & 64) hipLaunchKernelGGL((conv_h2s_kernel<4, 1>), grid, dim3(512), 0, s, a);
-        else if (a.tune & 8) hipLaunchKernelGGL((conv_h2s_kernel<4, 0, 4>), grid, dim3(512), 0, s, a);
-        else hipLaunchKernelGGL((conv_h2s_kernel<4, 0, 2>), grid, dim3(512), 0, s, a);
-    } else if (a.tune & 64) hipLaunchKernelGGL((conv_h2s_kernel<2, 1>), grid, dim3(256), 0, s, a);
-    else if (a.tune & 8) hipLaunchKernelGGL((conv_h2s_kernel<2, 0, 3>), grid, dim3(256), 0, s, a);
-    else hipLaunchKernelGGL((conv_h2s_kernel<2, 0, 2>), grid, dim3(256), 0, s, a);
+        if ((a.tune & 64) && (a.tune & 4096)) hipLaunchKernelGGL((conv_h2s_kernel<4, 7>), grid, dim3(512), 0, s, a, vmax);
+        else if ((a.tune & 64) && (a.tune & 2048)) hipLaunchKernelGGL((conv_h2s_kernel<4, 6>), grid, dim3(512), 0, s, a, vmax);
+        else if ((a.tune & 64) && (a.tune & 1024)) hipLaunchKernelGGL((conv_h2s_kernel<4, 5>), grid, dim3(512), 0, s, a, vmax);
+        else if ((a.tune & 64) && (a.tune & 256) && (a.tune & 512)) hipLaunchKernelGGL((conv_h2s_kernel<4, 4>), grid, dim3(512), 0, s, a, vmax);
+        else if ((a.tune & 64) && (a.tune & 256)) hipLaunchKernelGGL((conv_h2s_kernel<4, 2>), grid, dim3(512), 0, s, a, vmax);
+        else if ((a.tune & 64) && (a.tune & 512)) hipLaunchKernelGGL((conv_h2s_kernel<4, 3>), grid, dim3(512), 0, s, a, vmax);
+        else if (a.tune & 64) hipLaunchKernelGGL((conv_h2s_kernel<4, 1>), grid, dim3(512), 0, s, a, vmax);
+        else if (a.tune & 8) {
+            if (walk) hipLaunchKernelGGL((conv_h2s_kernel<4, 0, 4, 2, true>), grid, dim3(512), 0, s, a, vmax);
+            else hipLaunchKernelGGL((conv_h2s_kernel<4, 0, 4>), grid, dim3(512), 0, s, a, vmax);
+        } else if (walk) hipLaunchKernelGGL((conv_h2s_kernel<4, 0, 2, 2, true>), grid, dim3(512), 0, s, a, vmax);
+        else hipLaunchKernelGGL((conv_h2s_kernel<4, 0, 2>), grid, dim3(512), 0, s, a, vmax);
+    } else if (a.tune & 64) hipLaunchKernelGGL((conv_h2s_kernel<2, 1>), grid, dim3(256), 0, s, a, vmax);
+    else if (a.tune & 8) {
+        if (walk) hipLaunchKernelGGL((conv_h2s_kernel<2, 0, 3, 2, true>), grid, dim3(256), 0, s, a, vmax);
+        else hipLaunchKernelGGL((conv_h2s_kernel<2, 0, 3>), grid, dim3(256), 0, s, a, vmax);
+    } else if (walk) hipLaunchKernelGGL((conv_h2s_kernel<2, 0, 2, 2, true>), grid, dim3(256), 0, s, a, vmax);
+    else hipLaunchKernelGGL((conv_h2s_kernel<2, 0, 2>), grid, dim3(256), 0, s, a, vmax);
     return hipGetLastError();
 }
 
diff --git a/padel_analytics_amd/csrc/conv_patch_h2v.hip b/padel_analytics_amd/csrc/conv_patch_h2v.hip
--- a/padel_analytics_amd/csrc/conv_patch_h2v.hip
+++ b/padel_analytics_amd/csrc/conv_patch_h2v.hip
@@ -16,8 +16,26 @@
 
 }
 
-template <int NF, bool CHUNK, bool TAIL, bool WS>
-__global__ void __launch_bounds__(256, 2) conv_h2v_kernel(const ConvArgs a) {
+struct HvTile { int n, y0, x0, f0; bool valid; };
+__device__ __forceinline__ HvTile hv_tile(const ConvArgs& a, int v, int vmax, int nf) {
+    HvTile t;
+    const int nmt = a.n_mtiles, nnt = a.n_ntiles;
+    const int q8 = nmt >> 3, r8 = nmt & 7, xcd = v & 7, idx = v >> 3;
+    const int mloc = idx / nnt, nt = idx - mloc * nnt;
+    t.valid = v < vmax && mloc < q8 + (xcd < r8 ? 1 : 0);
+    const int mt = (xcd < r8 ? xcd * (q8 + 1) : r8 * (q8 + 1) + (xcd - r8) * q8) + mloc;
+    const int txN = (a.Wo + 15) >> 4, tyN = (a.Ho + 15) >> 4;
+    const int tpi = tyN * txN;
+    t.n = mt / tpi;
+    const int rt = mt - t.n * tpi;
+    const int ty = rt / txN, tx = rt - ty * txN;
+    t.y0 = ty * 16; t.x0 = tx * 16;
+    t.f0 = nt * nf;
+    return t;
+}
+
+template <int NF, bool CHUNK, bool TAIL, bool WS, bool WALK>
+__global__ void __launch_bounds__(256, 2) conv_h2v_kernel(const ConvArgs a, const int vmax) {
     static_assert(CHUNK || TAIL, "cin = 32 CHUNK + 16 TAIL");
     static_assert(WS || NF <= 2, "three products: 2 fragments per wave (6 register sets of 4 VGPRs per step)");
     constexpr int MF = 4;
@@ -31,69 +49,55 @@
     const int tid = threadIdx.x;
     const int lane = tid & 63;
     const int wave = __builtin_amdgcn_readfirstlane(tid >> 6);
-    const int lr = lane & 15, lq = lane >> 4;
-
-    const int nmt = a.n_mtiles, nnt = a.n_ntiles;
-    const int bid = blockIdx.x;
-    const int q8 = nmt >> 3, r8 = nmt & 7, xcd = bid & 7, idx = bid >> 3;
-    const int mloc = idx / nnt, nt = idx - mloc * nnt;
-    if (mloc >= q8 + (xcd < r8 ? 1 : 0)) return;
-    const int mt = (xcd < r8 ? xcd * (q8 + 1) : r8 * (q8 + 1) + (xcd - r8) * q8) + mloc;
-    const int txN = (a.Wo + 15) >> 4, tyN = (a.Ho + 15) >> 4;
-    const int tpi = tyN * txN;
-    const int n = mt / tpi, rt = mt - n * tpi;
-    const int ty = rt / txN, tx = rt - ty * txN;
-    const int y0 = ty * 16, x0 = tx * 16;
-    const int f0 = nt * NF;
-
-    const float* const in0 = a.in + (((long long)n * a.H + (y0 - 1)) * a.W + (x0 - 1)) * a.in_cs + a.in_choff;
-    const i32x4 rsrcP = make_rsrc3(in0);
+    const int G = (int)gridDim.x;
+    int v = (int)blockIdx.x;
+    HvTile cur = hv_tile(a, v, vmax, NF);
+    if (!cur.valid) return;
     const unsigned lp0 = __builtin_amdgcn_readfirstlane((unsigned)(uintptr_t)lds);
 
-    if constexpr (CHUNK) {
-        const int p_lane = lane >> 2;
-        const int p_q = (lane & 3) ^ (((lane >> 4) & 1) << 1);
-        const unsigned p_piece = (unsigned)((p_q >> 1) * 64 + (p_q & 1) * 16);
 #define PADEL_HV_PSPAN(S_)                                                                                        \
-        if (((S_) & 3) == wave) {                                                                                 \
-            const int pp_ = (S_) * 16 + p_lane;                                                                   \
-            const int py_ = pp_ / kVPW, px_ = pp_ - py_ * kVPW;                                                   \
-            const bool ok_ = pp_ < kVNPix && (unsigned)(y0 - 1 + py_) < (unsigned)a.H && (unsigned)(x0 - 1 + px_) < (unsigned)a.W; \
-            const unsigned vo_ = ok_ ? (unsigned)((py_ * a.W + px_) * a.in_cs * 4) + p_piece : kOOR3;             \
-            dma3<(S_) * 1024>(vo_, rsrcP, 0u, lp0);                                                               \
-            dma3<kVPlaneB + (S_) * 1024>(vo_, rsrcP, 32u, lp0);                                                   \
-        }
-        PADEL_HV_PSPAN(0) PADEL_HV_PSPAN(1) PADEL_HV_PSPAN(2) PADEL_HV_PSPAN(3) PADEL_HV_PSPAN(4) PADEL_HV_PSPAN(5) PADEL_HV_PSPAN(6)
-        PADEL_HV_PSPAN(7) PADEL_HV_PSPAN(8) PADEL_HV_PSPAN(9) PADEL_HV_PSPAN(10) PADEL_HV_PSPAN(11) PADEL_HV_PSPAN(12) PADEL_HV_PSPAN(13)
-        PADEL_HV_PSPAN(14) PADEL_HV_PSPAN(15) PADEL_HV_PSPAN(16) PADEL_HV_PSPAN(17) PADEL_HV_PSPAN(18) PADEL_HV_PSPAN(19) PADEL_HV_PSPAN(20)
-#undef PADEL_HV_PSPAN
+    if (((S_) & 3) == wave) {                                                                                     \
+        const int pp_ = (S_) * 16 + p_lane;                                                                       \
+        const int py_ = pp_ / kVPW, px_ = pp_ - py_ * kVPW;                                                       \
+        const bool ok_ = pp_ < kVNPix && (unsigned)(y0_ - 1 + py_) < (unsigned)a.H && (unsigned)(x0_ - 1 + px_) < (unsigned)a.W; \
+        const unsigned vo_ = ok_ ? (unsigned)((py_ * a.W + px_) * a.in_cs * 4) + p_piece : kOOR3;                 \
+        dma3<(S_) * 1024>(vo_, rsrcP_, 0u, lp0);                                                                  \
+        dma3<kVPlaneB + (S_) * 1024>(vo_, rsrcP_, 32u, lp0);                                                      \
     }
-    if constexpr (TAIL) {
-        const int t_lane = lane >> 1;
-        const unsigned t_piece = (unsigned)(((lane & 1) ^ ((lane >> 4) & 1)) * 16);
-        const unsigned t_so = CHUNK ? 128u : 0u;
 #define PADEL_HV_TSPAN(S_)                                                                                        \
-        if (((S_) & 3) == ((wave + 1) & 3)) {                                                                     \
-            const int pp_ = (S_) * 32 + t_lane;                                                                   \
-            const int py_ = pp_ / kVPW, px_ = pp_ - py_ * kVPW;                                                   \
-            const bool ok_ = pp_ < kVNPix && (unsigned)(y0 - 1 + py_) < (unsigned)a.H && (unsigned)(x0 - 1 + px_) < (unsigned)a.W; \
-            const unsigned vo_ = ok_ ? (unsigned)((py_ * a.W + px_) * a.in_cs * 4) + t_piece : kOOR3;             \
-            dma3<PATCH_B + (S_) * 1024>(vo_, rsrcP, t_so, lp0);                                                   \
-            dma3<PATCH_B + kVTPlaneB + (S_) * 1024>(vo_, rsrcP, t_so + 32u, lp0);                                 \
-        }
-        PADEL_HV_TSPAN(0) PADEL_HV_TSPAN(1) PADEL_HV_TSPAN(2) PADEL_HV_TSPAN(3) PADEL_HV_TSPAN(4) PADEL_HV_TSPAN(5)
-        PADEL_HV_TSPAN(6) PADEL_HV_TSPAN(7) PADEL_HV_TSPAN(8) PADEL_HV_TSPAN(9) PADEL_HV_TSPAN(10)
-#undef PADEL_HV_TSPAN
+    if (((S_) & 3) == ((wave + 1) & 3)) {                                                                         \
+        const int pp_ = (S_) * 32 + t_lane;                                                                       \
+        const int py_ = pp_ / kVPW, px_ = pp_ - py_ * kVPW;                                                       \
+        const bool ok_ = pp_ < kVNPix && (unsigned)(y0_ - 1 + py_) < (unsigned)a.H && (unsigned)(x0_ - 1 + px_) < (unsigned)a.W; \
+        const unsigned vo_ = ok_ ? (unsigned)((py_ * a.W + px_) * a.in_cs * 4) + t_piece : kOOR3;                 \
+        dma3<PATCH_B + (S_) * 1024>(vo_, rsrcP_, t_so, lp0);                                                      \
+        dma3<PATCH_B + kVTPlaneB + (S_) * 1024>(vo_, rsrcP_, t_so + 32u, lp0);                                    \
     }
+#define PADEL_HV_PATCH(T_)                                                                                        \
+    do {                                                                                                          \
+        const int y0_ = (T_).y0, x0_ = (T_).x0;                                                                   \
+        int ln_ = lane;                                                                                           \
+        if constexpr (WALK) asm volatile("" : "+v"(ln_));                                                         \
+        const int p_lane = ln_ >> 2, p_q = (ln_ & 3) ^ (((ln_ >> 4) & 1) << 1);                                   \
+        const unsigned p_piece = (unsigned)((p_q >> 1) * 64 + (p_q & 1) * 16);                                    \
+        const int t_lane = ln_ >> 1;                                                                              \
+        const unsigned t_piece = (unsigned)(((ln_ & 1) ^ ((ln_ >> 4) & 1)) * 16);                                 \
+        constexpr unsigned t_so = CHUNK ? 128u : 0u;                                                              \
+        (void)p_lane; (void)p_piece; (void)t_lane; (void)t_piece; (void)t_so;                                     \
+        const i32x4 rsrcP_ = make_rsrc3(a.in + (((long long)(T_).n * a.H + (y0_ - 1)) * a.W + (x0_ - 1)) * a.in_cs + a.in_choff); \
+        if constexpr (CHUNK) {                                                                                    \
+            PADEL_HV_PSPAN(0) PADEL_HV_PSPAN(1) PADEL_HV_PSPAN(2) PADEL_HV_PSPAN(3) PADEL_HV_PSPAN(4) PADEL_HV_PSPAN(5) PADEL_HV_PSPAN(6) \
+            PADEL_HV_PSPAN(7) PADEL_HV_PSPAN(8) PADEL_HV_PSPAN(9) PADEL_HV_PSPAN(10) PADEL_HV_PSPAN(11) PADEL_HV_PSPAN(12) PADEL_HV_PSPAN(13) \
+            PADEL_HV_PSPAN(14) PADEL_HV_PSPAN(15) PADEL_HV_PSPAN(16) PADEL_HV_PSPAN(17) PADEL_HV_PSPAN(18) PADEL_HV_PSPAN(19) PADEL_HV_PSPAN(20) \
+        }                                                                                                         \
+        if constexpr (TAIL) {                                                                                     \
+            PADEL_HV_TSPAN(0) PADEL_HV_TSPAN(1) PADEL_HV_TSPAN(2) PADEL_HV_TSPAN(3) PADEL_HV_TSPAN(4) PADEL_HV_TSPAN(5) \
+            PADEL_HV_TSPAN(6) PADEL_HV_TSPAN(7) PADEL_HV_TSPAN(8) PADEL_HV_TSPAN(9) PADEL_HV_TSPAN(10)            \
+        }                                                                                                         \
+    } while (0)
 
     constexpr unsigned fragb = (unsigned)NSTEPS * 2048u;
-    const unsigned voffW = (unsigned)lane * 16u;
     i32x4 rsrcW[NF];
-#pragma unroll
-    for (int j = 0; j < NF; ++j) {
-        const int frag = min(f0 + j, a.n16 - 1);
-        rsrcW[j] = make_rsrc3(reinterpret_cast<const char*>(a.wr) + (long long)frag * fragb);
-    }
     hv_i32x4 w[3][NF], wm[3][WS ? 1 : NF];
 #define PADEL_HV_LOADW(ST_)                                                                                       \
     do {                                                                                                          \
@@ -122,20 +126,8 @@
     } while (0)
 
     unsigned rbase[8];
-    if constexpr (CHUNK) {
-#pragma unroll
-        for (int r = 0; r < 8; ++r) {
-            const int p0 = 4 * wave * kVPW + lr;
-            rbase[r] = (unsigned)(p0 * 64 + ((lq ^ ((((p0 + r) >> 2) & 1) << 1)) << 4));
-        }
-    }
-    const int rd_pix = 4 * wave * kVPW + lr;
 
     f32x4 acc[MF][NF], part[MF][NF], cross[MF][NF];
-#pragma unroll
-    for (int f = 0; f < MF; ++f)
-#pragma unroll
-        for (int j = 0; j < NF; ++j) { acc[f][j] = (f32x4){0.f, 0.f, 0.f, 0.f}; part[f][j] = acc[f][j]; cross[f][j] = acc[f][j]; }
     h16x8 ah[4], am[4];
 #define PADEL_HV_READROW(R_, KX_)                                                                                 \
     do {                                                                                                          \
@@ -212,22 +204,73 @@
             _Pragma("unroll") for (int j = 0; j < NF; ++j) { acc[f][j] += part[f][j]; part[f][j] = (f32x4){0.f, 0.f, 0.f, 0.f}; } \
     } while (0)
 
-    PADEL_HV_LOADW(0);
-    if constexpr (NSTEPS > 1) PADEL_HV_LOADW(1);
-    wait_vm3<NW * (NSTEPS > 1 ? 2 : 1)>();
-    __builtin_amdgcn_s_barrier();
-    asm volatile("" ::: "memory");
-    if constexpr (CHUNK) {
-        PADEL_HV_READROW(0, 0); PADEL_HV_READROW(1, 0); PADEL_HV_READROW(2, 0); PADEL_HV_READROW(3, 0);
-        __builtin_amdgcn_sched_barrier(0);
-        PADEL_HV_STEP(0); PADEL_HV_STEP(1); PADEL_HV_STEP(2); PADEL_HV_STEP(3); PADEL_HV_STEP(4);
-        PADEL_HV_STEP(5); PADEL_HV_STEP(6); PADEL_HV_STEP(7); PADEL_HV_STEP(8);
-        PADEL_HV_FLUSH();
-    }
-    if constexpr (TAIL) {
-        constexpr int S0 = CHUNK ? 9 : 0;
-        PADEL_HV_TSTEP(0, S0); PADEL_HV_TSTEP(1, S0 + 1); PADEL_HV_TSTEP(2, S0 + 2); PADEL_HV_TSTEP(3, S0 + 3); PADEL_HV_TSTEP(4, S0 + 4);
-        PADEL_HV_FLUSH();
+    PADEL_HV_PATCH(cur);
+    for (;;) {
+        int ln = lane;
+        if constexpr (WALK) asm volatile("" : "+v"(ln));
+        const int lr = ln & 15, lq = ln >> 4;
+        const unsigned voffW = (unsigned)ln * 16u;
+        const int rd_pix = 4 * wave * kVPW + lr;
+        (void)rd_pix;
+#pragma unroll
+        for (int j = 0; j < NF; ++j) {
+            const int frag = min(cur.f0 + j, a.n16 - 1);
+            rsrcW[j] = make_rsrc3(reinterpret_cast<const char*>(a.wr) + (long long)frag * fragb);
+        }
+        PADEL_HV_LOADW(0);
+        if constexpr (NSTEPS > 1) PADEL_HV_LOADW(1);
+        HvTile nxt = {0, 0, 0, 0, false};
+        if constexpr (WALK) nxt = hv_tile(a, v + G, vmax, NF);
+        if constexpr (CHUNK) {
+            const int p0 = 4 * wave * kVPW + lr;
+#pragma unroll
+            for (int r = 0; r < 8; ++r) rbase[r] = (unsigned)(p0 * 64 + ((lq ^ ((((p0 + r) >> 2) & 1) << 1)) << 4));
+        }
+#pragma unroll
+        for (int f = 0; f < MF; ++f)
+#pragma unroll
+            for (int j = 0; j < NF; ++j) { acc[f][j] = (f32x4){0.f, 0.f, 0.f, 0.f}; part[f][j] = acc[f][j]; cross[f][j] = acc[f][j]; }
+        wait_vm3<NW * (NSTEPS > 1 ? 2 : 1)>();
+        __builtin_amdgcn_s_barrier();
+        asm volatile("" ::: "memory");
+        if constexpr (CHUNK) {
+            PADEL_HV_READROW(0, 0); PADEL_HV_READROW(1, 0); PADEL_HV_READROW(2, 0); PADEL_HV_READROW(3, 0);
+            __builtin_amdgcn_sched_barrier(0);
+            PADEL_HV_STEP(0); PADEL_HV_STEP(1); PADEL_HV_STEP(2); PADEL_HV_STEP(3); PADEL_HV_STEP(4);
+            PADEL_HV_STEP(5); PADEL_HV_STEP(6); PADEL_HV_STEP(7); PADEL_HV_STEP(8);
+            PADEL_HV_FLUSH();
+        }
+        if constexpr (TAIL) {
+            constexpr int S0 = CHUNK ? 9 : 0;
+            PADEL_HV_TSTEP(0, S0); PADEL_HV_TSTEP(1, S0 + 1); PADEL_HV_TSTEP(2, S0 + 2); PADEL_HV_TSTEP(3, S0 + 3); PADEL_HV_TSTEP(4, S0 + 4);
+            PADEL_HV_FLUSH();
+        }
+        if constexpr (WALK) {
+            if (nxt.valid) {
+                asm volatile("s_waitcnt lgkmcnt(0)" ::: "memory");
+                __builtin_amdgcn_s_barrier();
+                asm volatile("" ::: "memory");
+            }
+        }
+
+        int mpix[MF];
+#pragma unroll
+        for (int f = 0; f < MF; ++f) {
+            const int oy = cur.y0 + 4 * wave + f, ox = cur.x0 + lr;
+            mpix[f] = (oy < a.Ho && ox < a.Wo) ? (cur.n * a.Ho + oy) * a.Wo + ox : -1;
+        }
+        const bool fast = cur.y0 + 16 <= a.Ho && cur.x0 + 16 <= a.Wo && (cur.f0 + NF) * 16 <= a.cout && (((a.out_choff | a.out_cs) & 3) == 0) &&
+                          (!a.res || (((a.res_choff | a.res_cs) & 3) == 0));
+        if constexpr (WALK) {
+            h2_epilogue_walk<MF, NF>(a, acc, cross, mpix, cur.f0, lq, fast, [&]() {
+                if (nxt.valid) PADEL_HV_PATCH(nxt);
+            });
+        } else {
+            h2_epilogue<MF, NF>(a, acc, cross, mpix, cur.f0, lq, fast);
+        }
+        if (!WALK || !nxt.valid) break;
+        cur = nxt;
+        v += G;
     }
 #undef PADEL_HV_FLUSH
 #undef PADEL_HV_TSTEP
@@ -237,16 +280,9 @@
 #undef PADEL_HV_READROW
 #undef PADEL_HV_WAITW
 #undef PADEL_HV_LOADW
-
-    int mpix[MF];
-#pragma unroll
-    for (int f = 0; f < MF; ++f) {
-        const int oy = y0 + 4 * wave + f, ox = x0 + lr;
-        mpix[f] = (oy < a.Ho && ox < a.Wo) ? (n * a.Ho + oy) * a.Wo + ox : -1;
-    }
-    const bool fast = y0 + 16 <= a.Ho && x0 + 16 <= a.Wo && (f0 + NF) * 16 <= a.cout && (((a.out_choff | a.out_cs) & 3) == 0) &&
-                      (!a.res || (((a.res_choff | a.res_cs) & 3) == 0));
-    h2_epilogue<MF, NF>(a, acc, cross, mpix, f0, lq, fast);
+#undef PADEL_HV_PATCH
+#undef PADEL_HV_TSPAN
+#undef PADEL_HV_PSPAN
 }
 
 bool conv_h2v_supported(const ConvArgs& a) {
@@ -259,10 +295,19 @@
     const int batch = a.M / (a.Ho * a.Wo);
     a.n_mtiles = batch * ((a.Ho + 15) / 16) * ((a.Wo + 15) / 16);
     a.n_ntiles = (a.n16 + NF - 1) / NF;
-    dim3 grid(8u * (unsigned)((a.n_mtiles + 7) / 8) * (unsigned)a.n_ntiles, 1, 1);
-    if (a.cin == 48) hipLaunchKernelGGL((conv_h2v_kernel<NF, true, true, WS>), grid, dim3(256), 0, s, a);
-    else if (a.cin == 32) hipLaunchKernelGGL((conv_h2v_kernel<NF, true, false, WS>), grid, dim3(256), 0, s, a);
-    else hipLaunchKernelGGL((conv_h2v_kernel<NF, false, true, WS>), grid, dim3(256), 0, s, a);
+    const int vmax = 8 * ((a.n_mtiles + 7) / 8) * a.n_ntiles;
+    const bool walk = !(a.tune & 4) && (a.cin == 48 || (a.tune & 16));
+    const int per = walk ? h2_walk_slots(2) : vmax;
+    dim3 grid((unsigned)(vmax < per ? vmax : per), 1, 1);
+#define PADEL_HV_LAUNCH(CHUNK_, TAIL_)                                                                            \
+    do {                                                                                                          \
+        if (walk) hipLaunchKernelGGL((conv_h2v_kernel<NF, CHUNK_, TAIL_, WS, true>), grid, dim3(256), 0, s, a, vmax);  \
+        else hipLaunchKernelGGL((conv_h2v_kernel<NF, CHUNK_, TAIL_, WS, false>), grid, dim3(256), 0, s, a, vmax); \
+    } while (0)
+    if (a.cin == 48) PADEL_HV_LAUNCH(true, true);
+    else if (a.cin == 32) PADEL_HV_LAUNCH(true, false);
+    else PADEL_HV_LAUNCH(false, true);
+#undef PADEL_HV_LAUNCH
     return hipGetLastError();
 }
 
diff --git a/padel_analytics_amd/csrc/h2_common.h b/padel_analytics_amd/csrc/h2_common.h
--- a/padel_analytics_amd/csrc/h2_common.h
+++ b/padel_analytics_amd/csrc/h2_common.h
@@ -60,6 +60,99 @@
     const h2_u32x2 s1 = __builtin_amdgcn_permlane16_swap(rr[1], rr[3], false, false);
     const h2_u32x2 hd = {s0[0], s1[0]}, md = {s0[1], s1[1]};
     return h2_decode4(__builtin_bit_cast(h16x4, hd), __builtin_bit_cast(h16x4, md));
+}
+
+static inline int h2_walk_slots(int per_cu) {
+    static int n_cu = 0;
+    if (!n_cu) {
+        int dev = 0;
+        hipDeviceProp_t p;
+        if (hipGetDevice(&dev) == hipSuccess && hipGetDeviceProperties(&p, dev) == hipSuccess) n_cu = p.multiProcessorCount;
+        if (n_cu <= 0) n_cu = 256;
+    }
+    return (per_cu * n_cu) & ~7;
+}
+
+template <int MF, int NF>
+struct H2PairOps {
+    f32x4 b[NF], sc[NF];
+    h2_u32x4 rr[MF][NF];
+};
+template <int MF, int NF, bool RES>
+__device__ __forceinline__ void h2_pair_load(const ConvArgs& a, const int (&mpix)[MF], int fw, int lq, H2PairOps<MF, NF>& o) {
+#pragma unroll
+    for (int j = 0; j < NF; ++j) {
+        const int co0 = (fw + j) * 16 + lq * 4;
+        o.b[j] = *reinterpret_cast<const f32x4*>(a.bias + co0);
+        o.sc[j] = *reinterpret_cast<const f32x4*>(a.oscale + co0);
+    }
+    const int piece = ((lq & 1) << 5) | ((lq >> 1) << 4);
+#pragma unroll
+    for (int f = 0; f < MF; ++f) {
+        if constexpr (RES) {
+            const char* rp = reinterpret_cast<const char*>(a.res) + (long long)mpix[f] * a.res_cs * 4 + ((((a.res_choff >> 4) + fw) << 6) + piece);
+#pragma unroll
+            for (int j = 0; j < NF; ++j) o.rr[f][j] = *reinterpret_cast<const h2_u32x4*>(rp + j * 64);
+        }
+    }
+}
+template <int MF, int NF, bool RES>
+__device__ __forceinline__ void h2_pair_pin(H2PairOps<MF, NF>& o) {
+#pragma unroll
+    for (int j = 0; j < NF; ++j) {
+        asm volatile("" : "+v"(o.b[j]), "+v"(o.sc[j]) : : "memory");
+        if constexpr (RES) {
+#pragma unroll
+            for (int f = 0; f < MF; ++f) asm volatile("" : "+v"(o.rr[f][j]) : : "memory");
+        }
+    }
+}
+template <int MF, int NF, int ACT, bool RES>
+__device__ __forceinline__ void h2_pair_store(const ConvArgs& a, const f32x4 (&mainacc)[MF][NF], const f32x4 (&cross)[MF][NF],
+                                              const int (&mpix)[MF], int fw, int lq, const H2PairOps<MF, NF>& o, bool& bad) {
+    const int piece = ((lq & 1) << 5) | ((lq >> 1) << 4);
+    char* op[MF];
+#pragma unroll
+    for (int f = 0; f < MF; ++f)
+        op[f] = reinterpret_cast<char*>(a.out) + (long long)mpix[f] * a.out_cs * 4 + ((((a.out_choff >> 4) + fw) << 6) + piece);
+    h2_u16x2 top = {0, 0};
+#pragma unroll
+    for (int j = 0; j < NF; ++j)
+#pragma unroll
+        for (int f = 0; f < MF; ++f) {
+            f32x4 v;
+#pragma unroll
+            for (int r = 0; r < 4; ++r) v[r] = h2_conv_value(cross[f][j][r], mainacc[f][j][r], o.sc[j][r], o.b[j][r]);
+            if constexpr (RES) {
+                const f32x4 rv = h2_residual4(o.rr[f][j]);
+                if (a.res_pre) {
+#pragma unroll
+                    for (int r = 0; r < 4; ++r) v[r] = h2_act<ACT>(v[r] + rv[r]);
+                } else {
+#pragma unroll
+                    for (int r = 0; r < 4; ++r) v[r] = h2_act<ACT>(v[r]) + rv[r];
+                }
+            } else {
+#pragma unroll
+                for (int r = 0; r < 4; ++r) v[r] = h2_act<ACT>(v[r]);
+            }
+            h2_u32x2 hd, md;
+#pragma unroll
+            for (int p = 0; p < 2; ++p) {
+                const h2_f32x2 x = {__builtin_amdgcn_fmed3f(v[2 * p], -kH2Max, kH2Max), __builtin_amdgcn_fmed3f(v[2 * p + 1], -kH2Max, kH2Max)};
+                const h2_h16x2 hh = __builtin_convertvector(x, h2_h16x2);
+                const h2_f32x2 res = {(x[0] - (float)hh[0]) * kH2Scale, (x[1] - (float)hh[1]) * kH2Scale};
+                const h2_h16x2 mm = __builtin_convertvector(res, h2_h16x2);
+                hd[p] = __builtin_bit_cast(unsigned, hh);
+                md[p] = __builtin_bit_cast(unsigned, mm);
+                top = __builtin_elementwise_max(top, __builtin_bit_cast(h2_u16x2, hd[p] & 0x7FFF7FFFu));
+            }
+            const h2_u32x2 s0 = __builtin_amdgcn_permlane16_swap(hd[0], md[0], false, false);
+            const h2_u32x2 s1 = __builtin_amdgcn_permlane16_swap(hd[1], md[1], false, false);
+            const h2_u32x4 ov = {s0[0], s1[0], s0[1], s1[1]};
+            *reinterpret_cast<h2_u32x4*>(op[f] + j * 64) = ov;
+        }
+    bad = bad || top[0] >= 0x7BFFu || top[1] >= 0x7BFFu;
 }
 
 template <int MF, int NF, int ACT, bool RES, bool F32OUT>
@@ -207,4 +300,37 @@
     if (!a.out_f32) h2_raise(a.ovf_flag, bad);
 }
 
-}
+template <int MF, int NF, class IssueNext>
+__device__ __forceinline__ void h2_epilogue_walk(const ConvArgs& a, const f32x4 (&mainacc)[MF][NF], const f32x4 (&cross)[MF][NF],
+                                                 const int (&mpix)[MF], int fw, int lq, bool fast, IssueNext&& issue_next) {
+    const bool wide = fast && (a.out_f32 ? !a.res : ((((a.out_choff | a.out_cs) & 15) == 0) && (!a.res || (((a.res_choff | a.res_cs) & 15) == 0))));
+    const bool pairs = wide && !a.out_f32;
+    H2PairOps<MF, NF> o;
+    if (pairs && a.res) {
+        h2_pair_load<MF, NF, true>(a, mpix, fw, lq, o);
+        h2_pair_pin<MF, NF, true>(o);
+    } else if (pairs) {
+        h2_pair_load<MF, NF, false>(a, mpix, fw, lq, o);
+        h2_pair_pin<MF, NF, false>(o);
+    }
+    issue_next();
+    bool bad = false;
+#define PADEL_H2_EPI(ACT_)                                                                                        \
+    do {                                                                                                          \
+        if (pairs) {                                                                                              \
+            if (a.res) h2_pair_store<MF, NF, ACT_, true>(a, mainacc, cross, mpix, fw, lq, o, bad);                \
+            else h2_pair_store<MF, NF, ACT_, false>(a, mainacc, cross, mpix, fw, lq, o, bad);                     \
+        } else if (wide) h2_epilogue_fast<MF, NF, ACT_, false, true>(a, mainacc, cross, mpix, fw, lq, bad);       \
+        else if (a.res) h2_epilogue_slow<MF, NF, ACT_, true>(a, mainacc, cross, mpix, fw, lq, bad);               \
+        else h2_epilogue_slow<MF, NF, ACT_, false>(a, mainacc, cross, mpix, fw, lq, bad);                         \
+    } while (0)
+    if (a.act == ACT_SILU) PADEL_H2_EPI(ACT_SILU);
+    else if (a.act == ACT_RELU) PADEL_H2_EPI(ACT_RELU);
+    else if (a.act == ACT_SIGMOID) PADEL_H2_EPI(ACT_SIGMOID);
+    else if (a.act == ACT_LEAKY) PADEL_H2_EPI(ACT_LEAKY);
+    else PADEL_H2_EPI(ACT_NONE);
+#undef PADEL_H2_EPI
+    if (!a.out_f32) h2_raise(a.ovf_flag, bad);
+}
+
+}
```

Result: no change. 1023, median of 6 (+0.4%).
